# michalfratczak/habdec

Measured on AMD Instinct MI355X. Metric: IQ Msamples/s (batched 2.048 MS/s streams), higher is better.
Workload: dtype f32

## Files before the change

habdec_amd/capi.py:

```python
from __future__ import annotations

import ctypes as C
from pathlib import Path

import numpy as np

LIB_PATH = Path(__file__).resolve().parent / "libhabdec_amd.so"
_lib = None


class HabdecError(RuntimeError):
    pass


class hd_engine_config(C.Structure):
    _fields_ = [("device", C.c_int32), ("n_streams", C.c_uint32), ("max_chunk", C.c_uint32), ("sampling_rate", C.c_double),
                ("decimation", C.c_uint32), ("baud", C.c_double), ("rtty_bits", C.c_uint32), ("rtty_stops", C.c_float),
                ("lowpass_bw_hz", C.c_float), ("lowpass_trans", C.c_float), ("dc_remove", C.c_int32), ("lookup_mode", C.c_int32),
                ("enable_spectrum", C.c_int32), ("ungated", C.c_int32), ("keep_filtered", C.c_int32), ("pipeline", C.c_int32), ("arith", C.c_int32)]


class hd_afc_info(C.Structure):
    _fields_ = [("frequency_correction", C.c_double), ("shift_hz", C.c_double), ("noise_floor", C.c_double),
                ("noise_variance", C.c_double), ("peak_left", C.c_int32), ("peak_right", C.c_int32), ("spectra", C.c_uint64)]
# ... 40 lines not shown
    "hd_stream_set_dc_remove": (_int, [_vp, _u32, _int]),
    "hd_stream_reset_frequency_correction": (_int, [_vp, _u32, _dbl]),
    "hd_stream_set_tune": (_int, [_vp, _u32, _dbl]),
    "hd_stream_set_front_tune": (_int, [_vp, _u32, _dbl]),
    "hd_stream_front_tune": (_int, [_vp, _u32, C.POINTER(hd_front_tune_info)]),
    "hd_stream_set_auto_afc": (_int, [_vp, _u32, _int, _dbl, _dbl]),
    "hd_stream_tune": (_int, [_vp, _u32, C.POINTER(hd_tune_info)]),
    "hd_set_sentence_callback": (None, [_vp, SENTENCE_CB, _vp]),
    "hd_set_match_callback": (None, [_vp, MATCH_CB, _vp]),
    "hd_set_chars_callback": (None, [_vp, CHARS_CB, _vp]),
    "hd_process_host": (_int, [_vp, _vp, _sz, _vp, _u32]),
    "hd_process_device": (_int, [_vp, _vp, _sz, _vp, _u32]),
    "hd_flush": (_int, [_vp]),
    "hd_ingest_run": (_int, [_vp, _vp, C.c_uint64, C.POINTER(C.c_uint64)]),
    "hd_stream_rtty": (_sz, [_vp, _u32, C.c_char_p, _sz]),
    "hd_stream_last_sentence": (_sz, [_vp, _u32, C.c_char_p, _sz]),
    "hd_stream_take_sentences": (_sz, [_vp, _u32, C.c_char_p, _sz]),
    "hd_stream_take_matches": (_sz, [_vp, _u32, C.c_char_p, _sz]),
    "hd_stream_take_chars": (_sz, [_vp, _u32, C.c_char_p, _sz]),
    "hd_engine_sentences_ok": (C.c_uint64, [_vp]),
    "hd_stream_afc": (_int, [_vp, _u32, C.POINTER(hd_afc_info)]),
    "hd_stream_spectrum": (_sz, [_vp, _u32, _f32p, _sz]),
    "hd_stream_power": (_sz, [_vp, _u32, _f32p, _sz]),
    "hd_stream_demodulated": (_sz, [_vp, _u32, _f32p, _sz]),
    "hd_stream_decimated": (_sz, [_vp, _u32, _f32p, _sz]),
    "hd_stream_filtered": (_sz, [_vp, _u32, _f32p, _sz]),
    "hd_stream_bits": (_sz, [_vp, _u32, _u8p, _sz]),
    "hd_stream_flips": (_sz, [_vp, _u32, _u32p, _sz]),
    "hd_stream_fir_taps": (_sz, [_vp, _u32, _f32p, _sz]),
    "hd_stream_symbol_backlog": (_u32, [_vp, _u32]),
    "hd_stream_bits_total": (C.c_uint64, [_vp, _u32]),
    "hd_stream_flip_list_full": (C.c_uint64, [_vp, _u32]),
    "hd_stream_demod_checksum": (C.c_int, [_vp, _u32, C.POINTER(C.c_uint64), C.POINTER(C.c_uint32), C.POINTER(C.c_uint32)]),
    "hd_stream_demod_checksum_total": (C.c_int, [_vp, _u32, C.POINTER(C.c_uint64), C.POINTER(C.c_uint64), C.POINTER(C.c_uint64)]),
    "hd_min_chunk": (_u32, [_u32]),
    "hd_engine_timing": (_int, [_vp, C.POINTER(hd_timing)]),
    "hd_engine_set_timing": (None, [_vp, _int]),
}
HOST_API = {
    "hd_host_decim_plan": (_int, [C.c_uint, C.POINTER(_int), C.POINTER(C.c_uint)]),
    "hd_host_decim_taps": (_sz, [C.c_uint, _int, _f32p, _sz]),
    "hd_host_lowpass_design": (_sz, [_f, _f, _sz, _sz, _int, _f32p, _sz]),
    "hd_host_rtty_new": (_vp, [_sz, _f]),
    "hd_host_rtty_free": (None, [_vp]),
    "hd_host_rtty_pending": (_sz, [_vp]),
    "hd_host_rtty_push_run": (_sz, [_vp, _u8p, _sz, C.c_char_p, _sz]),
    "hd_host_crc16": (None, [C.c_char_p, _sz, C.c_char_p]),
    "hd_host_extract_sentence": (_int, [C.c_char_p, _sz, C.c_char_p, C.c_char_p, C.c_char_p, C.c_char_p, _sz]),
    "hd_host_text_new": (_vp, [_sz, _f]),
    "hd_host_text_free": (None, [_vp]),
    "hd_host_text_push_bits": (None, [_vp, _u8p, _sz]),
    "hd_host_text_get": (_sz, [_vp, _int, C.c_char_p, _sz]),
    "hd_host_afc_new": (_vp, []),
    "hd_host_afc_free": (None, [_vp]),
    "hd_host_afc_step": (None, [_vp, _int, _int, _int, _int, _f, _f, _dbl, _dbl, _sz, _dbl]),
    "hd_host_afc_reset": (None, [_vp, _dbl, _sz, _dbl]),
    "hd_host_afc_get": (None, [_vp] + [C.POINTER(_dbl)] * 4 + [C.POINTER(_int)] * 2),
    "hd_host_atan2f": (None, [_f32p, _f32p, _f32p, _sz]),
    "hd_host_discriminate": (None, [_f32p, _sz, _f, _f, _f32p]),
    "hd_host_spectrum_payload": (_sz, [_f32p, _sz, _dbl, _dbl, _dbl, _dbl, _int, _int, _f, _int, _int, _u8p, _sz, C.POINTER(_sz)]),
    "hd_host_demod_payload": (_sz, [_f32p, _sz, _int, _int, _u8p, _sz, C.POINTER(_sz)]),
    "hd_host_parse_time": (_int, [C.c_char_p, C.POINTER(_int), C.POINTER(_int), C.POINTER(_f)]),
    "hd_host_parse_gps_pos": (_int, [C.c_char_p, C.POINTER(_f)]),
    "hd_host_parse_sentence": (_int, [C.c_char_p, _vp]),
    "hd_host_timestamp_from_hms": (_sz, [C.c_int64, _int, _int, _f, C.c_char_p, _sz]),
    "hd_host_gps_distance": (None, [_dbl] * 6 + [C.POINTER(_dbl)]),
    "hd_host_sondehub_new": (_vp, [C.c_char_p, C.c_char_p]),
    "hd_host_sondehub_free": (None, [_vp]),
    "hd_host_sondehub_push_sentence": (_int, [_vp, _u32, C.c_char_p, C.c_char_p, C.c_int64]),
    "hd_host_sondehub_push": (_int, [_vp, C.c_char_p, C.c_char_p, C.c_char_p, _int, _f, _f, _f]),
    "hd_host_sondehub_size": (_sz, [_vp]),
    "hd_host_sondehub_take": (_sz, [_vp, C.c_int64, C.c_char_p, _sz, C.POINTER(_sz)]),
    "hd_host_utc_iso": (_sz, [C.c_int64, C.c_char_p, _sz]),
    "hd_host_json_number": (_sz, [_dbl, C.c_char_p, _sz]),
    "hd_host_iqfiles_open": (_vp, [C.POINTER(C.c_char_p), C.c_uint32, _int, C.c_uint32, C.c_uint32, _dbl]),
    "hd_host_iqfiles_close": (None, [_vp]),
    "hd_host_iqfiles_streams": (C.c_uint32, [_vp]),
    "hd_host_iqfiles_count": (C.c_uint64, [_vp, C.c_uint32]),
    "hd_host_iqfiles_rewinds": (C.c_uint64, [_vp, C.c_uint32]),
    "hd_host_iqfiles_next": (C.c_uint32, [_vp, _f32p, _sz, C.POINTER(C.c_uint32)]),
    "hd_host_tune_step": (_int, [_dbl, _dbl, C.POINTER(C.c_uint32)]),
    "hd_host_tune_tables": (None, [_f32p, _f32p]),
    "hd_host_tune_rotate": (None, [_f32p, _sz, C.c_uint32, C.c_uint32, _f32p]),
}


def lib() -> C.CDLL:
    global _lib
    if _lib is None:
        if not LIB_PATH.exists():
            raise HabdecError(f"{LIB_PATH} is missing: build it with `python -m habdec_amd.build` (hipcc, gfx950). "
                              "habdec_amd has no CPU or PyTorch fallback for the data path.")
        L = C.CDLL(str(LIB_PATH))
        for table in (ENGINE_API, HOST_API):
            for name, (res, args) in table.items():
                f = getattr(L, name)
                f.restype, f.argtypes = res, args
        _lib = L
    return _lib


def check(rc: int) -> None:
    if rc != 0:
        raise HabdecError(f"habdec_amd error {rc}: {lib().hd_last_error().decode()}")
```

habdec_amd/csrc/dev_types.h:

```cpp
#pragma once
#include <stdint.h>
#ifndef __HIPCC__
#ifndef __host__
#define __host__
#define __device__
#endif
#endif

namespace hd {

constexpr int kFftBins = 4096;
constexpr uint32_t kVentLimit = 30000;
constexpr uint32_t kFirBatch = 256;

struct StreamCall {
    uint32_t n_in;
    uint32_t n1;
    uint32_t n2;
    uint32_t zero_hist1;
    uint32_t zero_hist2;
    uint32_t pend_before;
    uint32_t fft_fill;
    uint32_t fft_take;
    uint32_t fft_run;
    uint32_t fir_m;
    uint32_t fir_taps;
    uint32_t fir_zero_hist;
    uint32_t pend_after;
    uint32_t dc_remove;
    uint32_t clear_pending;
    uint32_t fir_taps_prev;
};
__host__ __device__ inline uint32_t sc_taps_prev(const StreamCall& c) { return c.fir_taps_prev & 0xFFFFu; }
__host__ __device__ inline uint32_t sc_head_n(const StreamCall& c) { return (c.fir_taps_prev >> 16) & 0x3FFFu; }
__host__ __device__ inline bool sc_head_prev(const StreamCall& c) { return (c.fir_taps_prev >> 30) & 1u; }
__host__ __device__ inline bool sc_head_save(const StreamCall& c) { return (c.fir_taps_prev >> 31) & 1u; }
__host__ __device__ inline uint32_t sc_pack_taps_prev(uint32_t taps_prev, uint32_t head_n, bool head_prev, bool head_save)
{ return (taps_prev & 0xFFFFu) | ((head_n & 0x3FFFu) << 16) | ((head_prev ? 1u : 0u) << 30) | ((head_save ? 1u : 0u) << 31); }


struct SymbolParams {
    uint32_t spb;
    uint32_t R;
    uint32_t min_held;
    uint32_t float_abs;
    uint32_t reset;
};

struct SymState {
    uint32_t base;
    uint32_t held;
    uint32_t cached;
    uint32_t run_pos;
    float    run_sum;
    uint32_t _pad[3];
};

struct BitsHeader {
    uint32_t nbits;
    uint32_t held_after;
    uint32_t nflips;
    uint32_t overflow;
    uint32_t uncached;
    uint32_t demod_ck[2];
    uint32_t demod_n;
    uint32_t seq;
    uint32_t _pad[3];
};
static_assert(sizeof(BitsHeader) == 48, "result slot header");

struct SpectrumStatsDev {
    int32_t valid;
    int32_t peak1, peak2;
    float power1, power2;
    uint32_t seq;
    double mean, sigma;
};

}
```

habdec_amd/csrc/engine.cpp:

```cpp
#include <hip/hip_runtime.h>
#include <rocfft/rocfft.h>

#include <algorithm>
#include <atomic>
#include <chrono>
#include <cmath>
#include <cstdio>
#include <cstdlib>
#include <cstring>
#include <memory>
#include <condition_variable>
#include <mutex>
#include <thread>
#include <string>
#include <vector>

#include "../../include/habdec_amd.h"
#include "dev_types.h"
#include "host/afc_tracker.hpp"
#include "host/decim_plan.hpp"
#include "host/fir_design.hpp"
#include "host/iq_file_batch.hpp"
#include "host/text_stage.hpp"
#include "host/tune_host.hpp"
// ... 44 lines not shown
struct SizeState {
    size_t stage_buf[2] = {0, 0};
    size_t pending = 0;
    size_t fft_fill = 0;
    size_t fir_buf = 0;
    uint32_t fir_T_run = 0;
    uint32_t head_n = 0;
    uint64_t head_call = ~0ull;
    bool head_aside = false;
    uint32_t tune_phase = 0;
    uint32_t front_phase = 0;
    uint32_t win_ub = 0, inflight_m = 0;
    uint32_t last_n2 = 0, last_pend_before = 0, last_m = 0;
    int last_buf = 0;
};

struct StreamHost {
    double baud = 300;
    float lp_bw = 1500, lp_trans = 0.025f;
    bool dc = false;
    hd::LowpassDesigner lp;
    bool taps_dirty = false;
    uint32_t tune_step = 0;
    uint32_t held = 0;
    bool sym_reset = true;
    hd::TextStage text;
    hd::AfcTracker afc;
    hd::SpectrumStats stats{};
    bool have_spectrum = false;
    uint64_t spectra = 0;
    uint32_t last_nbits = 0, last_nflips = 0;
    uint64_t flip_list_full = 0;
    uint64_t bits_total = 0;
    std::vector<uint32_t> last_words;
    uint32_t demod_ck[2] = {0, 0}, demod_ck_n = 0xFFFFFFFFu;
    uint64_t demod_ck_call = 0;
    uint64_t demod_ck_hash = 0xCBF29CE484222325ull;
    uint64_t demod_ck_calls = 0, demod_ck_unknown = 0;
    double tune_hz = 0;
    uint64_t tune_from = 0, retunes = 0;
    bool auto_afc = false;
    double afc_hold_s = 6.0, afc_min_hz = 100.0;
    uint64_t afc_elapsed = 0;
    double front_hz = 0;
    uint32_t front_step = 0;
    uint64_t front_from = 0;
};

}

struct hd_engine {
    hd_engine_config cfg{};
    double fs = 0, fsd = 0;
    std::vector<hd::DecimStage> stages;
    uint32_t S = 0, D = 1;
    uint32_t n1_cap = 0, n2_cap = 0;
    uint32_t taps_cap = 0, fir_hist_cap = 0;
    size_t fbuf_stride = 0;
    uint32_t tail_cap = 0, backlog_cap = 0, slot_words = 0, flips_cap = 0, max_R = 0, min_R = 4;
    int bins_sep = 8;
    bool decode_enabled = true;
    bool fast = false;
    bool one_stream = false;
    bool no_tail = false;
    uint32_t tail_max_n2 = 2048;
    int last_route = -1;
    struct PendingTail { bool valid = false; hd::TailArgs ta{}; int slot = 0; int r2 = 0, t2 = 0; } pend;
    DevBuf<float2> fft_tw;
    bool no_claim = false;
    uint32_t step_run = 0;
    bool no_cu_step = false;
    uint32_t ring_run = 0;
    uint32_t ring_short_pct = 25;
    static constexpr uint32_t kS1Loaders = 2;
#ifndef HD_S1_SLOTS_BATCH
#define HD_S1_SLOTS_BATCH 4
#endif
    static constexpr uint32_t kS1Slots = HD_S1_SLOTS_BATCH;
    PinBuf<unsigned int> ring_gave_up;
    std::string fail_cause;
    bool device_failed = false;
    uint64_t step_launches = 0;
    DevBuf<unsigned int> step_ctr;
    uint32_t pend_max_taps = 0;
    bool dec_wgs_forced = false;
#ifdef HD_TIMING_EXPERIMENT
    int cu_exp = 0;
#else
    static constexpr int cu_exp = 0;
#endif
    uint32_t n_cus = 0, dec_wgs_per_cu = 0;
    hipStream_t qa = nullptr, qb = nullptr, qc = nullptr;
    hipStream_t qh = nullptr;
    DevBuf<float2> staging2;
    hipEvent_t ev_copy[2] = {nullptr, nullptr}, ev_staging_free[2] = {nullptr, nullptr};
    bool staging_used[2] = {false, false};
    uint64_t host_calls = 0, host_calls_in_place = 0;
    uint32_t timing_every = 8;
    hd_timing last_timing{};
    static constexpr uint32_t kLpFftMinTaps = 1024;
    uint32_t lpf_N[2] = {0, 0};
    rocfft_plan lpf_fwd[2] = {nullptr, nullptr}, lpf_inv[2] = {nullptr, nullptr};
    rocfft_execution_info lpf_info = nullptr;
    DevBuf<char> lpf_workbuf;
    DevBuf<float2> lpf_x, lpf_k;
    PinBuf<uint32_t> lpf_ntaps;
    uint32_t lpf_k_N = 0;
    bool lpf_k_stale = true;
    uint64_t lpf_calls = 0;

    DevBuf<float2> staging, dec1, dec1b, dec1c, hist1[2], hist2[2], fbuf[3], fft_in, spec, filtered;
    DevBuf<float> stage_taps[2], lp_taps, power, demod, tail, weight;
    DevBuf<unsigned long long> flipmask;
    DevBuf<uint32_t> flips_dbg;
    DevBuf<hd::SymState> d_symstate;
    DevBuf<hd::DemodCarry> carry[2];
    DevBuf<float2> fir_head;
    DevBuf<float> tune_tab;
    DevBuf<uint32_t> demod_ck_acc;
    uint32_t head_cap = 0;
    DevBuf<hd::SymbolParams> d_sym;
    PinBuf<hd::SymbolParams> h_sym;
    static constexpr int kSlots = 4;
    struct CallSlot {
        DevBuf<hd::StreamCall> d_call;
        PinBuf<hd::StreamCall> h_call;
        PinBuf<uint32_t> h_slots;
        PinBuf<hd::SpectrumStatsDev> h_stats;
        PinBuf<uint2> h_tune;
        PinBuf<uint2> h_front;
        bool timed = false, timed_step = false;
        hipEvent_t ev_front = nullptr, ev_done = nullptr, ev_params = nullptr, ev_spec = nullptr, t0 = nullptr, t1 = nullptr, t2 = nullptr, t3 = nullptr;
        bool busy = false;
        uint32_t seq = 0;
        uint64_t total_in = 0;
        uint32_t r1 = 1;
        ~CallSlot() { for (hipEvent_t ev : {ev_front, ev_done, ev_params, ev_spec, t0, t1, t2, t3}) if (ev) (void)hipEventDestroy(ev); }
    } slot[kSlots];
    uint64_t calls = 0;
    uint64_t delivered = 0;
    int cur = 0;
    int hist_cur = 0;
    int carry_cur = 0;
    bool sym_dirty = true;

    std::vector<StreamHost> st;
    std::vector<SizeState> mirror, mirror_next;
    std::recursive_mutex mtx;
    bool in_callback = false;
    hd_sentence_cb sentence_cb = nullptr; void* sentence_user = nullptr;
    hd_match_cb match_cb = nullptr; void* match_user = nullptr;
    hd_chars_cb chars_cb = nullptr; void* chars_user = nullptr;
    uint64_t sentences_ok = 0;

    ~hd_engine()
    {
        for (rocfft_plan pl : {lpf_fwd[0], lpf_fwd[1], lpf_inv[0], lpf_inv[1]}) if (pl) rocfft_plan_destroy(pl);
        if (lpf_info) rocfft_execution_info_destroy(lpf_info);
        if (qa) (void)hipStreamDestroy(qa);
        if (qb && qb != qa) (void)hipStreamDestroy(qb);
        if (qc && qc != qa) (void)hipStreamDestroy(qc);
        if (qh) (void)hipStreamDestroy(qh);
        for (hipEvent_t ev : {ev_copy[0], ev_copy[1], ev_staging_free[0], ev_staging_free[1]}) if (ev) (void)hipEventDestroy(ev);
    }
};

namespace {

std::once_flag g_rocfft_once;

hd::SymbolParams symbol_params(const hd_engine* e, const StreamHost& s)
{
    hd::SymbolParams p{};
    p.float_abs = e->cfg.lookup_mode ? 1u : 0u;
    p.min_held = 0xFFFFFFFFu;
    p.spb = 0; p.R = 4;
    if (e->fsd > 0 && s.baud > 0) {
        const double spb = std::round(e->fsd / s.baud);
        if (spb >= 1 && spb < 1e9) {
            p.spb = (uint32_t)spb;
            p.R = (uint32_t)std::max(4, int(p.spb / 4));
            p.min_held = (uint32_t)std::ceil(e->fsd / s.baud * 3);
        }
    }
    return p;
}

float cutoff_rel(const hd_engine* e, const StreamHost& s) { return (float)(s.lp_bw / e->fsd); }

int check_stream(const hd_engine* e, uint32_t s)
{
    if (!e) return fail(HD_ERR_INVALID, "null engine");
    if (s >= e->S) return fail(HD_ERR_INVALID, "stream index out of range");
    return HD_OK;
}

}

extern "C" {

const char* hd_last_error(void) { return g_err.c_str(); }

uint32_t hd_min_chunk(uint32_t decimation)
{
    std::vector<hd::DecimStage> st;
    if (!hd::decim_plan(decimation, st)) return 0;
    uint64_t need = decimation ? decimation : 1;
    uint64_t r = 1;
    for (const auto& g : st) { need = std::max<uint64_t>(need, (uint64_t)(g.taps.size() - 1) * r); r *= (uint64_t)g.ratio; }
    const uint64_t d = decimation ? decimation : 1;
    return (uint32_t)((need + d - 1) / d * d);
}

void hd_engine_config_default(hd_engine_config* c)
// ... 24 lines not shown
    e->fsd = e->fs / (double)e->D;
    e->decode_enabled = cfg->ungated || !(e->fsd > 4 * 40e3);
    if (cfg->baud > 0 && e->fsd / cfg->baud < 3.5)
        return fail(HD_ERR_UNSUPPORTED, "symbol rate above a third of the decimated rate (fewer than 4 samples per bit): the symbol extractor's windows would overlap");
    {
        const float rel = (float)(500.0f / e->fsd);
        e->bins_sep = std::max(8, (int)std::round((double)rel * (double)hd::kFftBins));
    }

    int ndev = 0;
    if (hipGetDeviceCount(&ndev) != hipSuccess || ndev <= cfg->device || cfg->device < 0)
        return fail(HD_ERR_DEVICE, "no HIP device " + std::to_string(cfg->device) + " (this library has no CPU path)");
    HD_HIP(hipSetDevice(cfg->device));
    HD_HIP(hipStreamCreateWithFlags(&e->qa, hipStreamNonBlocking));
    e->one_stream = cfg->pipeline == 0;
    e->no_tail = getenv("HD_NO_TAIL") != nullptr;
    e->no_claim = getenv("HD_NO_CLAIM") != nullptr;
    if (const char* v = getenv("HD_STEP_RUN")) e->step_run = (uint32_t)atoi(v);
    e->no_cu_step = getenv("HD_NO_CU_STEP") != nullptr;
    if (const char* v = getenv("HD_RING_RUN")) e->ring_run = (uint32_t)atoi(v);
    if (const char* v = getenv("HD_RING_SHORT_PCT")) e->ring_short_pct = std::min<uint32_t>((uint32_t)atoi(v), 100u);
    if (const char* v = getenv("HD_TAIL_MAX_N2")) e->tail_max_n2 = (uint32_t)strtoul(v, nullptr, 0);
    {
        hipDeviceProp_t prop;
        HD_HIP(hipGetDeviceProperties(&prop, cfg->device));
        e->n_cus = (uint32_t)prop.multiProcessorCount;
        e->dec_wgs_per_cu = cfg->pipeline ? 6u : 8u;
        if (const char* v = getenv("HD_DEC_WGS_PER_CU")) { e->dec_wgs_per_cu = (uint32_t)atoi(v); e->dec_wgs_forced = true; }
#ifdef HD_TIMING_EXPERIMENT
        if (const char* v = getenv("HD_CU_EXP")) e->cu_exp = atoi(v);
#endif
    }
    for (hipEvent_t* ev : {&e->ev_copy[0], &e->ev_copy[1], &e->ev_staging_free[0], &e->ev_staging_free[1]}) HD_HIP(hipEventCreateWithFlags(ev, hipEventDisableTiming));
    if (e->one_stream) e->qb = e->qc = e->qa;
    else {
        if (!e->qb) HD_HIP(hipStreamCreateWithFlags(&e->qb, hipStreamNonBlocking));
        HD_HIP(hipStreamCreateWithFlags(&e->qc, hipStreamNonBlocking));
    }
    for (auto& sl : e->slot) {
        static const unsigned ev_flags = (unsigned)hipEventDisableSystemFence;
        HD_HIP(hipEventCreateWithFlags(&sl.ev_front, hipEventDisableTiming | ev_flags));
        HD_HIP(hipEventCreateWithFlags(&sl.ev_done, hipEventDisableTiming | ev_flags));
        HD_HIP(hipEventCreateWithFlags(&sl.ev_params, hipEventDisableTiming | ev_flags));
        HD_HIP(hipEventCreateWithFlags(&sl.ev_spec, hipEventDisableTiming | ev_flags));
        for (hipEvent_t* ev : {&sl.t0, &sl.t1, &sl.t2, &sl.t3}) HD_HIP(hipEventCreateWithFlags(ev, ev_flags));
    }

    const uint32_t S = e->S;
    const uint32_t r0 = e->stages.size() > 0 ? e->stages[0].ratio : 1;
    e->n1_cap = cfg->max_chunk / r0;
    e->n2_cap = cfg->max_chunk / e->D;
    const uint32_t m_cap = ((e->n2_cap + hd::kFirBatch - 1) / hd::kFirBatch) * hd::kFirBatch + hd::kFirBatch;
    e->taps_cap = (m_cap | 1u) + 1u;
    e->fir_hist_cap = (e->taps_cap + 1u) & ~1u;
    e->fbuf_stride = (size_t)e->fir_hist_cap + hd::kFirBatch + e->n2_cap + 2;
    e->fbuf_stride = (e->fbuf_stride + 1) & ~(size_t)1;
    e->backlog_cap = hd::kVentLimit + 1 + m_cap;
    e->tail_cap = 1u;
    while (e->tail_cap < hd::kVentLimit + 1 + m_cap + 1024) e->tail_cap <<= 1;

    e->st.resize(S);
    e->mirror.resize(S);
    e->mirror_next.resize(S);
    for (auto& s : e->st) {
        s.baud = cfg->baud; s.lp_bw = cfg->lowpass_bw_hz; s.lp_trans = cfg->lowpass_trans; s.dc = cfg->dc_remove != 0;
        s.text.framer.nbits = cfg->rtty_bits; s.text.framer.nstops = cfg->rtty_stops;
        s.lp.float_trig = cfg->lookup_mode != 0;
    }
    {
        const hd::SymbolParams p = symbol_params(e.get(), e->st[0]);
        const uint32_t spb = std::max<uint32_t>(p.spb, 1);
        uint32_t bits = 3u * e->backlog_cap / spb + 64u;
        bits = std::max<uint32_t>(256u, (bits + 31u) & ~31u);
        e->slot_words = (uint32_t)(sizeof(hd::BitsHeader) / 4) + bits / 32;
        e->max_R = std::max<uint32_t>(p.R, 4);
        e->min_R = e->max_R;
    }
    e->flips_cap = cfg->keep_filtered ? 256 : 0;

    HD_HIP(e->staging.alloc((size_t)S * cfg->max_chunk));
    if (e->stages.size() == 2) for (auto* b : {&e->dec1, &e->dec1b, &e->dec1c}) HD_HIP(b->alloc((size_t)S * e->n1_cap));
    HD_HIP(e->step_ctr.alloc(2 * 16 * 32 + 32));
    HD_HIP(e->ring_gave_up.alloc(4));
    e->ring_gave_up.p[0] = 0;
    if (!e->no_claim && e->n_cus % 32u == 0) {
        const uint32_t n_xcd = e->n_cus / 32u;
        HD_HIP(hipDeviceSynchronize());
        const uint32_t seen = HDK(probe_xcc_mask, e->qa, e->n_cus, e->step_ctr.p + 2 * 16 * 32);
        if (n_xcd > 16 || seen != (n_xcd >= 32 ? 0xFFFFFFFFu : (1u << n_xcd) - 1u)) e->no_claim = true;
    } else
        e->no_claim = true;
    if (e->stages.size() >= 1) {
        for (auto& h : e->hist1) HD_HIP(h.alloc((size_t)S * (e->stages[0].taps.size() - 1)));
        HD_HIP(e->stage_taps[0].alloc(e->stages[0].taps.size() + 1));
        HD_HIP(hipMemcpy(e->stage_taps[0].p, e->stages[0].taps.data(), e->stages[0].taps.size() * 4, hipMemcpyHostToDevice));
    }
    if (e->stages.size() == 2) {
        for (auto& h : e->hist2) HD_HIP(h.alloc((size_t)S * (e->stages[1].taps.size() - 1)));
        HD_HIP(e->stage_taps[1].alloc(e->stages[1].taps.size() + 1));
        HD_HIP(hipMemcpy(e->stage_taps[1].p, e->stages[1].taps.data(), e->stages[1].taps.size() * 4, hipMemcpyHostToDevice));
    }
    for (auto& b : e->fbuf) HD_HIP(b.alloc((size_t)S * e->fbuf_stride));
    HD_HIP(e->lp_taps.alloc((size_t)S * e->taps_cap));
    HD_HIP(e->demod.alloc((size_t)S * m_cap));
    if (cfg->keep_filtered) HD_HIP(e->filtered.alloc((size_t)S * m_cap));
    HD_HIP(e->tail.alloc((size_t)S * e->tail_cap));
    HD_HIP(e->weight.alloc((size_t)S * e->tail_cap));
    HD_HIP(e->flipmask.alloc((size_t)S * (e->tail_cap / 64)));
    HD_HIP(e->d_symstate.alloc(S));
    if (e->flips_cap) HD_HIP(e->flips_dbg.alloc((size_t)S * e->flips_cap));
    for (auto& c : e->carry) HD_HIP(c.alloc(S));
    e->head_cap = std::min<uint32_t>(e->taps_cap, 8192u);
    HD_HIP(e->fir_head.alloc((size_t)S * e->head_cap));
    HD_HIP(e->demod_ck_acc.alloc((size_t)2 * S));
    HD_HIP(e->d_sym.alloc(S));
    HD_HIP(e->h_sym.alloc(S));
    for (auto& sl : e->slot) {
        HD_HIP(sl.d_call.alloc(S));
        HD_HIP(sl.h_call.alloc(S));
        HD_HIP(sl.h_slots.alloc((size_t)S * e->slot_words));
        HD_HIP(sl.h_tune.alloc(S));
        HD_HIP(sl.h_front.alloc(S));
    }
    {
        std::vector<float> tab(4 * hd::kTuneTable);
        hd::tune_tables(tab.data(), tab.data() + 2 * hd::kTuneTable);
        HD_HIP(e->tune_tab.alloc(tab.size()));
        HD_HIP(hipMemcpy(e->tune_tab.p, tab.data(), tab.size() * sizeof(float), hipMemcpyHostToDevice));
    }
    if (cfg->enable_spectrum) {
        HD_HIP(e->fft_in.alloc((size_t)S * hd::kFftBins));
        HD_HIP(e->spec.alloc((size_t)S * hd::kFftBins));
        HD_HIP(e->power.alloc((size_t)S * hd::kFftBins));
        for (auto& sl : e->slot) HD_HIP(sl.h_stats.alloc(S));
        {
            std::vector<float2> tw(hd::kFftBins);
            for (size_t m = 0; m < hd::kFftBins; ++m) {
                const double a = 2.0 * 3.14159265358979323846264338327950288 * (double)m / (double)hd::kFftBins;
                tw[m] = make_float2((float)std::cos(a), (float)-std::sin(a));
            }
            HD_HIP(e->fft_tw.alloc(hd::kFftBins));
            HD_HIP(hipMemcpy(e->fft_tw.p, tw.data(), tw.size() * sizeof(float2), hipMemcpyHostToDevice));
        }
    }
    if (e->fast && e->taps_cap >= hd_engine::kLpFftMinTaps && getenv("HD_NO_LP_FFT") == nullptr) {
        std::call_once(g_rocfft_once, [] { rocfft_setup(); });
        uint32_t N = 1;
        while (N < m_cap + e->taps_cap) N <<= 1;
        e->lpf_N[1] = N; e->lpf_N[0] = N / 2;
        size_t wmax = 0;
        for (int w = 0; w < 2; ++w) {
            const size_t len = e->lpf_N[w];
            if (rocfft_plan_create(&e->lpf_fwd[w], rocfft_placement_inplace, rocfft_transform_type_complex_forward, rocfft_precision_single, 1, &len, S, nullptr) != rocfft_status_success ||
                rocfft_plan_create(&e->lpf_inv[w], rocfft_placement_inplace, rocfft_transform_type_complex_inverse, rocfft_precision_single, 1, &len, S, nullptr) != rocfft_status_success)
                return fail(HD_ERR_DEVICE, "rocfft_plan_create (low-pass transforms) failed");
            for (rocfft_plan pl : {e->lpf_fwd[w], e->lpf_inv[w]}) { size_t wsz = 0; rocfft_plan_get_work_buffer_size(pl, &wsz); wmax = std::max(wmax, wsz); }
        }
        if (rocfft_execution_info_create(&e->lpf_info) != rocfft_status_success) return fail(HD_ERR_DEVICE, "rocfft_execution_info_create failed");
        if (wmax) { HD_HIP(e->lpf_workbuf.alloc(wmax)); rocfft_execution_info_set_work_buffer(e->lpf_info, e->lpf_workbuf.p, wmax); }
        HD_HIP(e->lpf_x.alloc((size_t)S * N));
        HD_HIP(e->lpf_k.alloc((size_t)S * N));
        HD_HIP(e->lpf_ntaps.alloc(S));
    }
    {
        hd_engine::CallSlot& sl = e->slot[0];
        hipStream_t q = e->qa;
// ... 138 lines not shown
int hd_stream_set_tune(hd_engine* e, uint32_t s, double offset_hz)
{
    if (int r = check_stream(e, s)) return r;
    std::lock_guard<std::recursive_mutex> l(e->mtx);
    uint32_t d = 0;
    if (!hd::tune_step(offset_hz, e->fsd, &d)) return fail(HD_ERR_INVALID, "tuning offset outside (-fs_dec/2, fs_dec/2)");
    StreamHost& st = e->st[s];
    st.tune_hz = offset_hz; st.tune_step = d; st.tune_from = e->calls;
    if (offset_hz == 0) e->mirror[s].tune_phase = 0;
    return HD_OK;
}
int hd_stream_set_front_tune(hd_engine* e, uint32_t s, double offset_hz)
{
    if (int r = check_stream(e, s)) return r;
    std::lock_guard<std::recursive_mutex> l(e->mtx);
    if (e->stages.empty()) return fail(HD_ERR_UNSUPPORTED, "an engine without a decimation stage has no input-rate tuning: hd_stream_set_tune is the same thing there");
    uint32_t d = 0;
    if (!hd::tune_step(offset_hz, e->fs, &d)) return fail(HD_ERR_INVALID, "tuning offset outside (-fs/2, fs/2)");
    StreamHost& st = e->st[s];
    st.front_hz = offset_hz; st.front_step = d; st.front_from = e->calls;
    if (offset_hz == 0) e->mirror[s].front_phase = 0;
    return HD_OK;
}
int hd_stream_front_tune(hd_engine* e, uint32_t s, hd_front_tune_info* out)
{
    if (int r = check_stream(e, s)) return r;
    if (!out) return fail(HD_ERR_INVALID, "null argument");
    std::lock_guard<std::recursive_mutex> l(e->mtx);
    const StreamHost& st = e->st[s];
    out->offset_hz = st.front_hz; out->step = st.front_step; out->phase = e->mirror[s].front_phase; out->from_call = st.front_from;
    return HD_OK;
}
int hd_stream_set_auto_afc(hd_engine* e, uint32_t s, int on, double hold_s, double min_hz)
{
    if (int r = check_stream(e, s)) return r;
    if (!(hold_s >= 0) || !(min_hz >= 0)) return fail(HD_ERR_INVALID, "hold_s and min_hz must be >= 0");
    std::lock_guard<std::recursive_mutex> l(e->mtx);
    StreamHost& st = e->st[s];
    st.auto_afc = on != 0; st.afc_hold_s = hold_s; st.afc_min_hz = min_hz; st.afc_elapsed = 0;
    return HD_OK;
}
int hd_stream_tune(hd_engine* e, uint32_t s, hd_tune_info* out)
{
    if (int r = check_stream(e, s)) return r;
    if (!out) return fail(HD_ERR_INVALID, "null argument");
    std::lock_guard<std::recursive_mutex> l(e->mtx);
    const StreamHost& st = e->st[s];
    out->offset_hz = st.tune_hz; out->step = st.tune_step; out->phase = e->mirror[s].tune_phase;
    out->retunes = st.retunes; out->from_call = st.tune_from; out->auto_afc = st.auto_afc ? 1 : 0;
    return HD_OK;
}

}


namespace {

int run_pending_tail(hd_engine* e)
{
    if (!e->pend.valid) return HD_OK;
    hd_engine::CallSlot& ps = e->slot[e->pend.slot];
    e->pend.valid = false;
    hd::TailArgs ta = e->pend.ta;
    const int lanes = (e->S >= 2 * e->n_cus ? 64 : 256);
    hd::TailArgs lay = ta;
    if (lanes != 64) {
        if (!HDK(tail_layout, lay, lanes, e->pend.r2, e->pend.t2, e->pend_max_taps, e->max_R, e->min_R, e->tail_cap, e->pend.ta.pend_max, 64 * 1024)) return fail(HD_ERR_INVALID, "stream tail layout");
    }
    if (!HDK(launch_tail, e->qa, lanes, e->pend.r2, e->pend.t2, e->S, lay, ps.ev_done)) return fail(HD_ERR_INVALID, "stream tail refused a shape it was selected for");
    HD_HIP(hipGetLastError());
    return HD_OK;
}

int collect(hd_engine* e, hd_engine::CallSlot& sl)
{
    if (!sl.busy) return HD_OK;
    if (e->pend.valid && &e->slot[e->pend.slot] == &sl) { if (const int r = run_pending_tail(e)) return r; }
    const auto w0 = std::chrono::steady_clock::now();
    HD_HIP(hipEventSynchronize(sl.ev_done));
    const auto w1 = std::chrono::steady_clock::now();
    sl.busy = false;
    if (sl.timed) {
        float a = 0, b = 0;
        HD_HIP(hipEventElapsedTime(&b, sl.t1, sl.t2));
        if (sl.timed_step) a = b; else HD_HIP(hipEventElapsedTime(&a, sl.t0, sl.t3));
        e->last_timing.ms_total = a;
        e->last_timing.ms_front = b;
        e->last_timing.samples = sl.total_in;
        e->last_timing.front_bytes = sl.total_in * 8 + (sl.total_in / sl.r1) * 8;
        ++e->last_timing.timed_calls;
    }
    int rc = HD_OK;
    {
        const auto t_lim = std::chrono::steady_clock::now() + std::chrono::milliseconds(200);
        const bool timing_experiment = e->cu_exp != 0;
        auto await = [&](const volatile uint32_t* tag, const char* what, uint32_t s) {
            for (uint32_t spins = 0; *tag != sl.seq; ++spins) {
                if (std::chrono::steady_clock::now() > t_lim) {
                    e->device_failed = true;
                    e->fail_cause = std::string(what) + " of stream " + std::to_string(s) + " does not carry its call's tag 200 ms after the completion event";
                    rc = fail(HD_ERR_DEVICE, e->fail_cause + ": the results of this engine are unreliable -- destroy the engine");
                    return;
                }
                if (spins > 64u) std::this_thread::yield();
            }
        };
        for (uint32_t s = 0; s < e->S && !e->device_failed && !timing_experiment; ++s) {
            await(&reinterpret_cast<const volatile hd::BitsHeader*>(sl.h_slots.p + (size_t)s * e->slot_words)->seq, "result slot", s);
            if (!e->device_failed && e->cfg.enable_spectrum && sl.h_stats.p && sl.h_call.p[s].fft_run)
                await(reinterpret_cast<const volatile uint32_t*>(&sl.h_stats.p[s].seq), "spectrum statistics", s);
        }
        std::atomic_thread_fence(std::memory_order_acquire);
    }
    if (e->ring_gave_up.p && e->ring_gave_up.p[0] && !e->device_failed) {
        e->device_failed = true;
        e->fail_cause = "k_stage1_cu (loader / consumer waves): a bounded wait ran out inside a launch (word " + std::to_string(e->ring_gave_up.p[0]) + ")";
    }
    if (e->device_failed && rc == HD_OK)
        rc = fail(HD_ERR_DEVICE, e->fail_cause + ": the results of this and of every later call of this engine are unreliable -- destroy the engine");
    if (e->device_failed) {
        e->last_timing.host_wait_us = std::chrono::duration<double, std::micro>(w1 - w0).count();
        e->last_timing.host_text_us = 0;
        return rc;
    }
    for (uint32_t s = 0; s < e->S; ++s) {
        StreamHost& st = e->st[s];
        const hd::StreamCall& c = sl.h_call.p[s];
        if (c.fft_run) {
            std::memcpy(&st.stats, &sl.h_stats.p[s], sizeof(st.stats));
            st.have_spectrum = true;
            ++st.spectra;
        }
        const bool past_batch_gate = c.fir_m || c.clear_pending;
        if (past_batch_gate && e->cfg.enable_spectrum) st.afc.step(st.have_spectrum, st.stats, hd::kFftBins, e->fsd);
        st.afc_elapsed += c.n_in;
        if (st.auto_afc && (double)st.afc_elapsed >= st.afc_hold_s * e->fs && std::abs(st.afc.correction) > st.afc_min_hz) {
            const double corr = st.afc.correction;
            uint32_t d = 0;
            if (hd::tune_step(st.tune_hz + corr, e->fsd, &d)) {
                st.tune_hz += corr; st.tune_step = d; st.tune_from = e->calls;
                if (!d) e->mirror[s].tune_phase = 0;
                st.afc.reset(corr, hd::kFftBins, e->fsd);
                st.afc_elapsed = 0;
                ++st.retunes;
            }
        }
        const uint32_t* slot = sl.h_slots.p + (size_t)s * e->slot_words;
        const hd::BitsHeader* hdr = reinterpret_cast<const hd::BitsHeader*>(slot);
        SizeState& sz = e->mirror[s];
        st.held = hdr->held_after;
        sz.inflight_m -= c.fir_m;
        sz.win_ub = hdr->uncached + sz.inflight_m;
        st.last_nbits = hdr->nbits; st.last_nflips = hdr->nflips;
        st.bits_total += hdr->nbits;
        st.demod_ck[0] = hdr->demod_ck[0]; st.demod_ck[1] = hdr->demod_ck[1]; st.demod_ck_n = hdr->demod_n; st.demod_ck_call = e->delivered;
        if (hdr->demod_n != 0xFFFFFFFFu) {
            for (const uint32_t x : {hdr->demod_n, hdr->demod_ck[0], hdr->demod_ck[1]}) st.demod_ck_hash = (st.demod_ck_hash ^ x) * 0x100000001B3ull;
            ++st.demod_ck_calls;
        } else ++st.demod_ck_unknown;
        if (hdr->overflow & 1u) rc = fail(HD_ERR_CAPACITY, "symbol result slot overflow on stream " + std::to_string(s));
        if (hdr->overflow & 2u) ++st.flip_list_full;
        const uint32_t* words = slot + sizeof(hd::BitsHeader) / 4;
        st.last_words.assign(words, words + (hdr->nbits + 31) / 32);
        if (!c.fir_m) continue;
        if (hdr->nbits) st.text.framer.push_packed(words, hdr->nbits);
        const std::string chars = st.text.run(hdr->nbits != 0, [&](const hd::SentenceMatch& m) {
            ++e->sentences_ok;
// ... 158 lines not shown
    const uint32_t step_lds = (p.R1 == 32 || p.R1 == 64) ? HDK(step_lds_bytes, (int)p.R1, (int)p.T1) : 0u;
    const bool step = tail && !p.any_front && e->cfg.pipeline && !e->one_stream && p.min_in == p.max_in && p.max_in && step_lds &&
                      HDK(tail_layout, r.ta_step, 64, R2, T2, p.max_taps, e->max_R, e->min_R, e->tail_cap, p.max_pend, step_lds);
    r.route = step ? Route::step : tail ? Route::tail : Route::separate;
    r.any_post = p.any_dc || (p.any_tune && !tail);
    r.lean = tail && !e->one_stream;
    r.free_front = !tail && p.nst == 2 && !e->one_stream;
    r.host_params = tail && !step && e->one_stream;
    r.dcall = r.host_params ? sl.h_call.dev : sl.d_call.p;
    r.feed = (e->cfg.enable_spectrum && !r.any_post) ? e->fft_in.p : nullptr;
    if (r.route != Route::separate || !e->cfg.enable_spectrum || r.any_post || !p.any_fft) return;
    for (uint32_t s = 0; s < S; ++s) {
        hd::StreamCall& c = sl.h_call.p[s];
        if (c.fft_run == 1 && c.fft_fill == 0 && c.fft_take == (uint32_t)hd::kFftBins) { c.fft_take = 0; c.fft_run = 2; }
    }
    r.spectrum_on_qc = !e->one_stream && p.nst != 0;
    for (uint32_t s = 0; s < S && r.spectrum_on_qc; ++s) r.spectrum_on_qc = sl.h_call.p[s].fft_run != 1u;
}

void fill_tail(const hd_engine* e, const hd_engine::CallSlot& sl, const CallPlan& p, const CallRoute& r, const CallBufs& b, hd::TailArgs& t)
{
    t.dec1 = b.d1; t.dec1_stride = e->n1_cap; t.hist2_in = e->hist2[b.hin].p; t.hist2_out = e->hist2[b.hout].p; t.taps2 = e->stage_taps[1].p;
    t.fbuf = b.fcur; t.fbuf_next = b.fnext; t.fbuf_stride = e->fbuf_stride; t.fir_hist_cap = e->fir_hist_cap;
    t.lp_taps = e->lp_taps.p; t.taps_stride = e->taps_cap; t.demod = e->demod.p; t.demod_stride = e->demod.n / e->S;
    t.filtered = e->cfg.keep_filtered ? e->filtered.p : nullptr; t.carry_in = e->carry[b.cin].p; t.carry_out = e->carry[b.cout].p;
    t.tune = p.any_tune ? sl.h_tune.dev : nullptr; t.tune_tab = e->tune_tab.p;
    t.call = r.dcall; t.fft_in = r.feed; t.head_buf = e->fir_head.p; t.fbuf_prev = b.fprev; t.head_cap = e->head_cap;
    t.n_streams = e->S;
    t.ring = e->tail.p; t.ring_cap = e->tail_cap; t.sym = e->d_symstate.p; t.flipmask = e->flipmask.p; t.wsum = e->weight.p;
    t.sp = e->d_sym.p; t.slots = sl.h_slots.dev; t.slot_words = e->slot_words; t.seq = sl.seq;
    t.flips_dbg = e->flips_cap ? e->flips_dbg.p : nullptr; t.flips_cap = e->flips_cap;
    t.fft_tw = r.feed ? e->fft_tw.p : nullptr;
    t.spec = e->spec.p; t.power = e->power.p; t.stats = sl.h_stats.dev; t.rate = e->fsd; t.bins_sep = e->bins_sep;
}

hd::StepClaim make_claim(const hd_engine* e, const CallPlan& p, uint32_t lin_wgs ,
                         uint32_t run_len_cu )
{
    hd::StepClaim claim{};
    const int R1 = (int)p.R1, T1 = (int)p.T1;
    const uint64_t S = e->S;
    const uint32_t ntiles = run_len_cu ? HDK(ring_tiles, R1, T1, p.max_in) : (p.max_n1 + 63) / 64, n_xcd = e->n_cus / 32u, run_len = run_len_cu ? run_len_cu : e->step_run >= 2 ? e->step_run : 4u;
    const uint64_t runs = S * ntiles / run_len;
    const bool shape_ok = run_len_cu ? (HDK(stage1_cu_supported, R1, T1) && p.max_in % 2048u == 0) : ((R1 == 32 || R1 == 64) && p.max_n1 % 64 == 0);
    if (!e->no_claim && (p.nst == 2 || (run_len_cu && p.nst == 1)) && shape_ok && p.min_in == p.max_in && p.max_in && !p.any_zero1 && n_xcd && e->n_cus % 32u == 0 && n_xcd <= 16 &&
        ntiles && (ntiles % run_len == 0 || (run_len_cu && R1 >= 32 && (S * ntiles) % run_len == 0)) && runs % n_xcd == 0 && S * ntiles < (1ull << 32) && (uint64_t)ntiles * S >= 4ull * lin_wgs) {
        claim.ctr = e->step_ctr.p + (size_t)(e->step_launches & 1u) * 16 * 32;
        claim.ctr_next = e->step_ctr.p + (size_t)((e->step_launches & 1u) ^ 1u) * 16 * 32;
        claim.n_xcd = n_xcd; claim.runs_per_xcd = (uint32_t)(runs / n_xcd); claim.run_len = run_len;
        if (run_len_cu && R1 >= 32 && e->ring_short_pct) {
            const uint32_t tpx = claim.runs_per_xcd * run_len, whole = (uint32_t)((uint64_t)tpx * (100u - e->ring_short_pct) / 100u) / run_len;
            claim.tiles_per_xcd = tpx; claim.short_from = whole; claim.runs_per_xcd = whole + (tpx - whole * run_len);
        }
    }
    return claim;
}

uint32_t pick_ring_run(const hd_engine* e, uint32_t R1, uint32_t ntiles)
{
    const uint64_t S = e->S;
    const uint32_t n_xcd = e->n_cus / 32u ? e->n_cus / 32u : 1u, want = R1 >= 32 ? 4u : 8u;
    auto ok = [&](uint32_t r) { return r >= 2u && r <= ntiles && (R1 >= 32 ? (S * ntiles) % r == 0 : ntiles % r == 0) && (S * ntiles / r) % n_xcd == 0; };
    if (e->ring_run >= 2 && ok(e->ring_run)) return e->ring_run;
    for (uint32_t d = 0; d <= 8u; ++d) {
        if (ok(want + d)) return want + d;
        if (d && d < want && ok(want - d)) return want - d;
    }
    return 2u;
}

int enqueue_uploads(hd_engine* e, hd_engine::CallSlot& sl, const CallRoute& r)
{
    const uint32_t S = e->S;
    hipStream_t qa = e->qa;
    if (e->last_route >= 0 && e->last_route != (int)r.route) {
        if (const int rc = run_pending_tail(e)) return rc;
        HD_HIP(hipStreamSynchronize(qa)); HD_HIP(hipStreamSynchronize(e->qb));
    }
    e->last_route = (int)r.route;
    e->last_timing.path = (uint32_t)r.route;
    if (!r.lean && !r.free_front && e->calls >= 2 && !e->one_stream) HD_HIP(hipStreamWaitEvent(qa, e->slot[(e->calls - 2) % hd_engine::kSlots].ev_done, 0));
    const bool step = r.route == Route::step;
    sl.timed = e->timing_every && (e->calls % e->timing_every) == 0;
    sl.timed_step = sl.timed && step;
    if (sl.timed && !step) HD_HIP(hipEventRecord(sl.t0, qa));
    if (!r.lean && !r.free_front && !r.host_params) {
        HDK(launch_fetch_params, e->qc, sl.h_call.dev, sl.d_call.p, S * sizeof(hd::StreamCall));
        if (!e->one_stream) { HD_HIP(hipEventRecord(sl.ev_params, e->qc)); HD_HIP(hipStreamWaitEvent(qa, sl.ev_params, 0)); }
    }
    for (uint32_t s = 0; s < S; ++s) {
        StreamHost& st = e->st[s];
        if (!st.taps_dirty) continue;
        HD_HIP(hipMemcpyAsync(e->lp_taps.p + (size_t)s * e->taps_cap, st.lp.taps.data(), st.lp.taps.size() * 4, hipMemcpyHostToDevice, qa));
        st.taps_dirty = false;
        e->lpf_k_stale = true;
    }
    if (e->sym_dirty) {
        uint32_t mr = 4;
        for (uint32_t s = 0; s < S; ++s) {
            e->h_sym.p[s] = symbol_params(e, e->st[s]);
            e->h_sym.p[s].reset = e->st[s].sym_reset ? 1u : 0u;
            mr = std::max(mr, e->h_sym.p[s].R);
        }
        e->max_R = mr;
        { uint32_t lo = mr; for (uint32_t s2 = 0; s2 < S; ++s2) lo = std::min(lo, std::max<uint32_t>(e->h_sym.p[s2].R, 4)); e->min_R = lo; }
        HD_HIP(hipMemcpyAsync(e->d_sym.p, e->h_sym.p, S * sizeof(hd::SymbolParams), hipMemcpyHostToDevice, qa));
        e->sym_dirty = false;
        for (uint32_t s = 0; s < S; ++s)
            if (e->st[s].sym_reset) { e->st[s].sym_reset = false; e->sym_dirty = true; }
    }
    return HD_OK;
}

int enqueue_step(hd_engine* e, hd_engine::CallSlot& sl, const CallPlan& p, CallRoute& r, const float2* iq, size_t stride)
{
    const uint32_t S = e->S;
    const int R1 = (int)p.R1, T1 = (int)p.T1, R2 = (int)p.R2, T2 = (int)p.T2;
    hipStream_t qa = e->qa;
    const CallBufs b = call_bufs(e);
    const uint32_t ring_nt = HDK(ring_tiles, R1, T1, p.max_in), ring_run = pick_ring_run(e, p.R1, ring_nt), n_xcd = e->n_cus / 32u;
    const bool runs_ok = ring_nt && n_xcd && ring_run >= 2u && ((uint64_t)S * ring_nt) % ring_run == 0 && ((uint64_t)S * ring_nt / ring_run) % n_xcd == 0;
    const bool cu_shape = !e->no_cu_step && !e->no_claim && !p.any_zero1 && p.max_in % 2048u == 0 && runs_ok && HDK(step_cu_supported, R1, T1, R2, T2);
    const uint32_t cu_tail = cu_shape ? HDK(step_cu_tail_lds, R1, T1) : 0u;
    if (cu_tail) {
        hd::TailArgs tacu{};
        if (HDK(tail_layout, tacu, 64, R2, T2, p.max_taps, e->max_R, e->min_R, e->tail_cap, p.max_pend, cu_tail)) r.ta_step = tacu;
    }
    fill_tail(e, sl, p, r, b, r.ta_step);
    hd_engine::PendingTail prev = e->pend;
    hd_engine::CallSlot* ps = prev.valid ? &e->slot[prev.slot] : nullptr;
    const int cu_exp = e->cu_exp;
    const bool want_cu = cu_tail && ((cu_exp & 1) || (r.ta_step.lds_bytes <= cu_tail && (!prev.valid || prev.ta.lds_bytes <= cu_tail)));
    const hd::StepClaim claim = make_claim(e, p, 0, want_cu ? ring_run : 0u);
    bool launched = false;
    if (want_cu && claim.ctr) {
        const uint32_t tb = std::max(r.ta_step.lds_bytes, prev.valid ? prev.ta.lds_bytes : 0u);
        hd::StepClaim cl = claim;
        if (cu_exp & 2) { cl.runs_per_xcd = 0; cl.tiles_per_xcd = 0; cl.short_from = 0xFFFFFFFFu; }
        launched = HDK(launch_step_cu, qa, R1, T1, prev.valid ? prev.r2 : R2, prev.valid ? prev.t2 : T2, S, e->n_cus, iq, stride,
                                      e->hist1[b.hin].p, e->hist1[b.hout].p, e->stage_taps[0].p, b.d1, e->n1_cap, sl.h_call.dev, sl.d_call.p, prev.ta,
                                      (prev.valid && !(cu_exp & 1)) ? S : 0u, p.max_in, cl, tb,
                                      sl.timed ? sl.t1 : nullptr, sl.timed ? sl.t2 : ps ? ps->ev_done : nullptr);
    }
    e->last_timing.step_variant = launched ? 1u : 0u;
    if (launched) ++e->step_launches;
    else {
        if (sl.timed) HD_HIP(hipEventRecord(sl.t1, qa));
        const hd::StepClaim fb = (want_cu && claim.ctr) ? hd::StepClaim{} : claim;
        const uint32_t wgs = (fb.ctr ? 8u : 32u) * e->n_cus;
        if (prev.valid && prev.ta.lds_bytes > HDK(step_lds_bytes, R1, T1)) {
            if (const int rc = run_pending_tail(e)) return rc;
            prev.valid = false; ps = nullptr;
        }
        if (!HDK(launch_step, qa, R1, T1, prev.valid ? prev.r2 : R2, prev.valid ? prev.t2 : T2, S, p.max_n1, iq, stride, e->hist1[b.hin].p,
                             e->hist1[b.hout].p, e->stage_taps[0].p, b.d1, e->n1_cap, sl.h_call.dev, sl.d_call.p, wgs, prev.ta, prev.valid ? S : 0u,
                             p.any_zero1 ? 0u : p.max_in, fb))
            return fail(HD_ERR_INVALID, "no step kernel for this decimation plan");
        if (fb.ctr) ++e->step_launches;
    }
    if (sl.timed && !launched) HD_HIP(hipEventRecord(sl.t2, qa));
    if (ps && (!launched || sl.timed)) HD_HIP(hipEventRecord(ps->ev_done, qa));
    HD_HIP(hipGetLastError());
    return HD_OK;
}

void call_spectrum(hd_engine* e, hipStream_t q, hd_engine::CallSlot& sl, const CallPlan& p, const CallRoute& r)
{
    if (!(e->cfg.enable_spectrum && p.max_n2)) return;
    const float2* fcur = e->fbuf[e->cur].p;
    if (r.any_post || p.nst == 0) HDK(launch_fft_feed, q, e->S, fcur, e->fbuf_stride, e->fft_in.p, r.dcall, e->fir_hist_cap);
    if (!p.any_fft) return;
    hd::launch_spectrum_wave(q, e->S, e->fft_in.p, e->fft_tw.p, e->spec.p, e->power.p, sl.h_stats.dev, r.dcall, e->fsd, e->bins_sep, sl.seq, fcur, e->fbuf_stride, e->fir_hist_cap);
}

int enqueue_front(hd_engine* e, hd_engine::CallSlot& sl, const CallPlan& p, const CallRoute& r, const float2* iq, size_t stride)
{
    const uint32_t S = e->S, R1 = p.R1, T1 = p.T1;
    const bool tail = r.route == Route::tail;
    hipStream_t qa = e->qa;
    const CallBufs b = call_bufs(e);
    if (p.nst == 0) {
        if (sl.timed) HD_HIP(hipEventRecord(sl.t1, qa));
        HDK(launch_passthrough, qa, S, p.max_in, iq, stride, b.fcur, e->fbuf_stride, r.dcall, e->fir_hist_cap);
        if (sl.timed) HD_HIP(hipEventRecord(sl.t2, qa));
    } else {
        const bool single = p.nst == 1;
        float2* out1 = single ? b.fcur : b.d1;
        const size_t out1_stride = single ? e->fbuf_stride : e->n1_cap;
        const uint32_t wgs_cu = (R1 == 64 && !e->dec_wgs_forced && e->dec_wgs_per_cu > 4u) ? 4u : e->dec_wgs_per_cu;
        const uint32_t lin1 = (p.min_in == p.max_in && p.max_in) ? wgs_cu * e->n_cus : 0u;
        bool s1_cu = false;
        if (!p.any_front && (single ? R1 == 4 : R1 != 4) && p.min_in == p.max_in && p.max_in && !e->no_cu_step && !p.any_zero1 && p.max_in % 2048u == 0 && HDK(stage1_cu_supported, (int)R1, (int)T1)) {
            const hd::StepClaim cl = make_claim(e, p, 0, pick_ring_run(e, R1, HDK(ring_tiles, (int)R1, (int)T1, p.max_in)));
            if (cl.ctr) {
                if (sl.timed) HD_HIP(hipEventRecord(sl.t1, qa));
                s1_cu = HDK(launch_stage1_cu, qa, (int)R1, (int)T1, e->n_cus, iq, stride, e->hist1[b.hin].p, e->hist1[b.hout].p, e->stage_taps[0].p, out1, out1_stride,
                                             p.max_in, cl, e->ring_gave_up.dev, hd_engine::kS1Loaders, 16u, (e->cfg.pipeline && !tail && !single) ? hd_engine::kS1Slots : 8u,
                                             single ? r.dcall : nullptr, e->fir_hist_cap, single ? r.feed : nullptr);
                if (s1_cu) ++e->step_launches;
            }
        }
        e->last_timing.step_variant = s1_cu ? 1u : 0u;
        if (!s1_cu) {
            if (sl.timed) HD_HIP(hipEventRecord(sl.t1, qa));
            const hd::StreamCall* call1 = (r.lean || r.free_front) ? sl.h_call.dev : r.dcall;
            if (!(p.any_front ? HDK(launch_decimate_tuned, qa, R1, T1, S, p.max_n1, iq, stride, e->hist1[b.hin].p, e->hist1[b.hout].p, e->stage_taps[0].p, out1, out1_stride,
                                                          call1, single ? 1 : 0, e->fir_hist_cap, single ? r.feed : nullptr, lin1, sl.h_front.dev, e->tune_tab.p)
                              : HDK(launch_decimate, qa, R1, T1, S, p.max_n1, iq, stride, e->hist1[b.hin].p, e->hist1[b.hout].p, e->stage_taps[0].p, out1, out1_stride,
                                                    call1, 0, single ? 1 : 0, e->fir_hist_cap, single ? r.feed : nullptr, lin1)))
                return fail(HD_ERR_INVALID, "no kernel for this decimation stage");
        }
        if (sl.timed) HD_HIP(hipEventRecord(sl.t2, qa));
        if (r.free_front) HDK(launch_fetch_params, qa, sl.h_call.dev, sl.d_call.p, S * sizeof(hd::StreamCall));
        if (!single && !tail) {
            if (!HDK(launch_decimate, qa, p.R2, p.T2, S, p.max_n2, b.d1, e->n1_cap, e->hist2[b.hin].p, e->hist2[b.hout].p, e->stage_taps[1].p, b.fcur,
                                     e->fbuf_stride, r.dcall, 1, 1, e->fir_hist_cap, r.feed))
                return fail(HD_ERR_INVALID, "no kernel for this decimation stage");
        }
    }
    if (!tail) {
        if (r.any_post) HDK(launch_chunk_post, qa, S, b.fcur, e->fbuf_stride, r.dcall, e->fir_hist_cap, p.any_tune ? sl.h_tune.dev : nullptr, e->tune_tab.p);
        if (!r.spectrum_on_qc) call_spectrum(e, qa, sl, p, r);
    }
    if (!e->one_stream) HD_HIP(hipEventRecord(sl.ev_front, qa));
    if (r.spectrum_on_qc) {
        HD_HIP(hipStreamWaitEvent(e->qc, sl.ev_front, 0));
        call_spectrum(e, e->qc, sl, p, r);
        HD_HIP(hipEventRecord(sl.ev_spec, e->qc));
    }
    return HD_OK;
}

int lowpass_transforms(hd_engine* e, const CallPlan& p, const CallRoute& r, const CallBufs& b, uint32_t* lpN)
{
    *lpN = 0;
    if (!e->fast || !e->lpf_N[1] || p.max_taps < hd_engine::kLpFftMinTaps || !p.max_m || p.any_lp_restart) return HD_OK;
    const uint32_t S = e->S, Lmax = p.max_m + p.max_taps - 1;
    const int w = Lmax <= e->lpf_N[0] ? 0 : Lmax <= e->lpf_N[1] ? 1 : -1;
    if (w < 0) return HD_OK;
    const uint32_t N = e->lpf_N[w];
    hipStream_t qb = e->qb;
    rocfft_execution_info_set_stream(e->lpf_info, qb);
    if (e->lpf_k_stale || e->lpf_k_N != N) {
        for (uint32_t s = 0; s < S; ++s) e->lpf_ntaps.p[s] = (uint32_t)e->st[s].lp.taps.size();
// ... 411 lines not shown
```

habdec_amd/csrc/host_api.cpp:

```cpp
#include <algorithm>
#include <cstring>
#include <string>

#include "../../include/habdec_amd_host.h"
#include "host/afc_tracker.hpp"
#include "host/decim_plan.hpp"
#include "host/fir_design.hpp"
#include "host/gui_payload.hpp"
#include "host/telemetry.hpp"
#include "host/sondehub.hpp"
#include "host/text_stage.hpp"
#include "host/iq_file_batch.hpp"
#include "host/tune_host.hpp"
#include "kernels/exact_math.h"

struct hd_host_rtty { hd::RttyFramer f; };
struct hd_host_text { hd::TextStage t; };
struct hd_host_afc { hd::AfcTracker a; };

static void put(char* dst, size_t cap, const std::string& s)
{
    if (!dst || !cap) return;
    const size_t n = std::min(cap - 1, s.size());
    std::memcpy(dst, s.data(), n);
    dst[n] = 0;
}

extern "C" {

int hd_host_decim_plan(unsigned total, int ratio[2], unsigned ntaps[2])
{
    std::vector<hd::DecimStage> st;
    if (!hd::decim_plan(total, st)) return -1;
    for (size_t i = 0; i < st.size(); ++i) { ratio[i] = st[i].ratio; ntaps[i] = (unsigned)st[i].taps.size(); }
    return (int)st.size();
}
size_t hd_host_decim_taps(unsigned total, int stage, float* taps, size_t cap)
{
    std::vector<hd::DecimStage> st;
    if (!hd::decim_plan(total, st) || stage < 0 || (size_t)stage >= st.size()) return 0;
    const auto& t = st[stage].taps;
    std::memcpy(taps, t.data(), std::min(cap, t.size()) * sizeof(float));
    return t.size();
}
size_t hd_host_lowpass_design(float cutoff_rel, float transition, size_t batch, size_t prev_ntaps, int float_trig, float* taps, size_t cap)
{
    hd::LowpassDesigner d;
    d.float_trig = float_trig != 0;
    d.batch = batch;
    d.taps.assign(prev_ntaps, 0.0f);
    if (!d.design(cutoff_rel, transition)) return 0;
    std::memcpy(taps, d.taps.data(), std::min(cap, d.taps.size()) * sizeof(float));
    return d.taps.size();
}

hd_host_rtty* hd_host_rtty_new(size_t nbits, float nstops) { auto* r = new hd_host_rtty; r->f.nbits = nbits; r->f.nstops = nstops; return r; }
void hd_host_rtty_free(hd_host_rtty* r) { delete r; }
size_t hd_host_rtty_pending(const hd_host_rtty* r) { return r ? r->f.pending() : 0; }
size_t hd_host_rtty_push_run(hd_host_rtty* r, const uint8_t* bits, size_t n, char* out, size_t cap)
{
    r->f.push_bits(bits, n);
    std::string s;
    r->f.frame(s);
    std::memcpy(out, s.data(), std::min(cap, s.size()));
    return s.size();
}

void hd_host_crc16(const char* s, size_t n, char out4[5])
{
    const std::string r = hd::crc16_ccitt_hex(std::string(s, n));
    std::memcpy(out4, r.c_str(), 5);
}
int hd_host_extract_sentence(const char* stream, size_t n, char* callsign, char* data, char* crc, char* rest, size_t cap)
{
    hd::SentenceMatch m;
    if (!hd::extract_sentence(std::string(stream, n), m)) return 0;
    put(callsign, cap, m.callsign); put(data, cap, m.data); put(crc, cap, m.crc); put(rest, cap, m.rest);
    return 1;
}

hd_host_text* hd_host_text_new(size_t nbits, float nstops) { auto* t = new hd_host_text; t->t.framer.nbits = nbits; t->t.framer.nstops = nstops; return t; }
void hd_host_text_free(hd_host_text* t) { delete t; }
void hd_host_text_push_bits(hd_host_text* t, const uint8_t* bits, size_t n)
{
    if (n) t->t.framer.push_bits(bits, n);
    t->t.run(n != 0, [](const hd::SentenceMatch&) {});
}
size_t hd_host_text_get(hd_host_text* t, int which, char* buf, size_t cap)
{
    const std::string* s = &t->t.stream;
    if (which == 1) s = &t->t.last_sentence; else if (which == 2) s = &t->t.ok_log; else if (which == 3) s = &t->t.match_log; else if (which == 4) s = &t->t.char_log;
    put(buf, cap, *s);
    return s->size();
}

hd_host_afc* hd_host_afc_new(void) { return new hd_host_afc; }
void hd_host_afc_free(hd_host_afc* a) { delete a; }
// ... 67 lines not shown
size_t hd_host_timestamp_from_hms(int64_t now_unix, int hour, int minute, float second, char* buf, size_t cap)
{
    const std::string s = hd::telemetry::timestamp_from_hms(now_unix, hour, minute, second);
    if (buf && cap) { const size_t n = std::min(cap - 1, s.size()); std::memcpy(buf, s.data(), n); buf[n] = 0; }
    return s.size();
}
void hd_host_gps_distance(double lat1, double lon1, double alt1, double lat2, double lon2, double alt2, double out[5])
{
    const auto d = hd::telemetry::gps_distance(lat1, lon1, alt1, lat2, lon2, alt2);
    out[0] = d.line; out[1] = d.circle; out[2] = d.radians; out[3] = d.elevation_deg; out[4] = d.bearing_deg;
}

struct hd_host_sondehub {
    hd::SondehubBatch b;
    std::string pending;
    size_t pending_n = 0;
    hd_host_sondehub(const char* u, const char* v) : b(u ? u : "", v ? v : "") {}
};
hd_host_sondehub* hd_host_sondehub_new(const char* uploader_callsign, const char* software_version) { return new hd_host_sondehub(uploader_callsign, software_version); }
void hd_host_sondehub_free(hd_host_sondehub* h) { delete h; }
int hd_host_sondehub_push_sentence(hd_host_sondehub* h, uint32_t stream, const char* callsign, const char* data, int64_t now_unix_ns)
{
    if (!h || !callsign || !data) return -1;
    return h->b.push_sentence(stream, callsign, data, now_unix_ns);
}
int hd_host_sondehub_push(hd_host_sondehub* h, const char* payload_callsign, const char* time_received, const char* datetime, int frame, float lat, float lon, float alt)
{
    if (!h || !payload_callsign || !time_received || !datetime) return -1;
    hd::SondeRecord r;
    r.payload_callsign = payload_callsign; r.time_received = time_received; r.datetime = datetime; r.frame = frame; r.lat = lat; r.lon = lon; r.alt = alt;
    h->b.push(r);
    return 1;
}
size_t hd_host_sondehub_size(const hd_host_sondehub* h) { return h ? h->b.size() : 0; }
size_t hd_host_sondehub_take(hd_host_sondehub* h, int64_t now_unix_ns, char* out, size_t cap, size_t* n_records)
{
    if (!h) return 0;
    if (h->pending.empty()) h->pending = h->b.take(now_unix_ns, &h->pending_n);
    const size_t n = h->pending.size();
    if (n_records) *n_records = h->pending_n;
    if (out && cap > n) { std::memcpy(out, h->pending.data(), n); out[n] = 0; h->pending.clear(); h->pending_n = 0; }
    return n;
}
size_t hd_host_utc_iso(int64_t unix_ns, char* buf, size_t cap)
{
    const std::string s = hd::utc_iso_ns(unix_ns);
    if (buf && cap) { const size_t n = std::min(cap - 1, s.size()); std::memcpy(buf, s.data(), n); buf[n] = 0; }
    return s.size();
}
size_t hd_host_json_number(double v, char* buf, size_t cap)
{
    const std::string s = hd::json_number(v);
    if (buf && cap) { const size_t n = std::min(cap - 1, s.size()); std::memcpy(buf, s.data(), n); buf[n] = 0; }
    return s.size();
}

hd_host_iqfiles* hd_host_iqfiles_open(const char* const* paths, uint32_t n_files, int loop, uint32_t chunk, uint32_t granule, double realtime_rate)
{
    if (!paths || !n_files) return nullptr;
    std::vector<std::string> v;
    for (uint32_t i = 0; i < n_files; ++i) { if (!paths[i]) return nullptr; v.emplace_back(paths[i]); }
    auto* h = new hd_host_iqfiles;
    if (!h->batch.open(v, loop != 0, chunk, granule, realtime_rate)) { delete h; return nullptr; }
    return h;
}
void hd_host_iqfiles_close(hd_host_iqfiles* h) { delete h; }
uint32_t hd_host_iqfiles_streams(const hd_host_iqfiles* h) { return h ? h->batch.streams() : 0; }
uint64_t hd_host_iqfiles_count(const hd_host_iqfiles* h, uint32_t stream) { return (h && stream < h->batch.streams()) ? h->batch.file(stream).count() : 0; }
uint64_t hd_host_iqfiles_rewinds(const hd_host_iqfiles* h, uint32_t stream) { return (h && stream < h->batch.streams()) ? h->batch.file(stream).rewinds() : 0; }
uint32_t hd_host_iqfiles_next(hd_host_iqfiles* h, float* slab, size_t stride, uint32_t* n_per_stream)
{
    if (!h || !slab || !n_per_stream || stride < h->batch.chunk()) return 0;
    return h->batch.next(slab, stride, n_per_stream);
}

int hd_host_tune_step(double offset_hz, double decimated_rate, uint32_t* step)
{
    uint32_t d = 0;
    if (!hd::tune_step(offset_hz, decimated_rate, &d)) return -1;
    if (step) *step = d;
    return 0;
}
void hd_host_tune_tables(float coarse[512], float fine[512]) { hd::tune_tables(coarse, fine); }
void hd_host_tune_rotate(const float* iq, size_t n, uint32_t phase, uint32_t step, float* out)
{
    float tab[4 * hd::kTuneTable];
    hd::tune_tables(tab, tab + 2 * hd::kTuneTable);
    hd::tune_rotate(tab, iq, n, phase, step, out);
}

}
```

habdec_amd/csrc/kernels/decimate.hip:

```cpp
#include <hip/hip_runtime.h>
#include <hip/hip_ext.h>
#include <type_traits>
#include <cstdlib>

#include "launch.h"
#include "tune.h"
#include "tail_body.h"
#include "stage1_ring.h"

#ifndef HD_FRONT_SWEEPS
#define HD_FRONT_SWEEPS 2
#endif
#define HD_DEC_MAXW 4

namespace hd {
namespace HD_ARITH_NS {

#ifdef HD_STAMP_DEC
#ifndef HD_STAMP_DEC_D
#define HD_STAMP_DEC_D 32
#endif
__device__ unsigned long long g_dec_stamps[4096 * 8];
extern "C" void HD_DBG_NAME(hd_debug_dec_stamps)(unsigned long long* host, size_t n) { (void)hipMemcpyFromSymbol(host, HIP_SYMBOL(g_dec_stamps), n * 8); }
#define DSTAMP_DECL unsigned long long ds_t = __builtin_amdgcn_s_memtime(), ds_acc[4] = {0, 0, 0, 0}; const unsigned long long ds_r0 = __builtin_amdgcn_s_memrealtime(); unsigned long long ds_r1 = 0
// ... 436 lines not shown
                leave_copy(s);
            }
        }
        if (jump) {
            __syncthreads();
            s = jump_s; tile_i = jump_first; jump = false;
            if constexpr (TUNED) ft.tn = ftune[s];
            if (!tile_i) leave_copy(s);
        }
    }
    store_prev();
    flush_copy();
    DSTAMP_WRITE();
}

template <int D, int T, int TO>
__global__ __launch_bounds__(TO) __attribute__((amdgpu_waves_per_eu(D == 64 ? 1 : 2, TO == 64 ? 2 : HD_DEC_MAXW))) void k_decimate(const float2* __restrict__ in, size_t in_stride,
                                                   const float2* __restrict__ hist_in, float2* __restrict__ hist_out,
                                                   const float* __restrict__ taps,
                                                   float2* __restrict__ out, size_t out_stride,
                                                   const StreamCall* __restrict__ call, int stage, int final_stage,
                                                   uint32_t fir_hist_cap, uint32_t tiles_per_wg, float2* __restrict__ fft_in,
                                                   uint32_t n_streams, uint32_t lin_ntiles, StreamCall* __restrict__ call_copy,
                                                   const uint32_t uniform_n, const StepClaim claim)
{
    __shared__ float4 tile4[dec_tile_f4<D, T, TO>()];
    decimate_body<D, T, TO>(in, in_stride, hist_in, hist_out, taps, out, out_stride, call, stage, final_stage, fir_hist_cap, tiles_per_wg, fft_in,
                            n_streams, lin_ntiles, call_copy, blockIdx.x, blockIdx.y, gridDim.x, tile4, TO == 64 ? uniform_n : 0u,
                            TO == 64 ? claim : StepClaim{});
}

template <int TO> constexpr bool front_tab_in_lds()
{
#ifdef HD_FRONT_TAB_GLOBAL
    return false;
#else
    return TO > 64;
#endif
}

template <int D, int T, int TO>
__global__ __launch_bounds__(TO) __attribute__((amdgpu_waves_per_eu(D == 64 ? 1 : 2, TO == 64 ? 2 : HD_DEC_MAXW))) void k_decimate_tuned(const float2* __restrict__ in, size_t in_stride,
                                                   const float2* __restrict__ hist_in, float2* __restrict__ hist_out,
                                                   const float* __restrict__ taps,
                                                   float2* __restrict__ out, size_t out_stride,
                                                   const StreamCall* __restrict__ call, int final_stage,
                                                   uint32_t fir_hist_cap, uint32_t tiles_per_wg, float2* __restrict__ fft_in,
                                                   uint32_t n_streams, uint32_t lin_ntiles,
                                                   const uint2* __restrict__ ftune, const float* __restrict__ ftab)
{
    constexpr bool kLds = front_tab_in_lds<TO>();
    __shared__ float4 tile4[dec_tile_f4<D, T, TO>()];
    __shared__ float4 tab4[kLds ? kTuneTable : 1];
    if constexpr (kLds) {
        for (uint32_t i = threadIdx.x; i < kTuneTable; i += TO) tab4[i] = reinterpret_cast<const float4*>(ftab)[i];
        __syncthreads();
    }
    decimate_body<D, T, TO, true>(in, in_stride, hist_in, hist_out, taps, out, out_stride, call, 0, final_stage, fir_hist_cap, tiles_per_wg, fft_in,
                                  n_streams, lin_ntiles, nullptr, blockIdx.x, blockIdx.y, gridDim.x, tile4, 0u, StepClaim{}, ftune,
                                  kLds ? reinterpret_cast<const float*>(tab4) : ftab);
}

template <int D, int T, int D2, int T2>
__global__ __launch_bounds__(64) __attribute__((amdgpu_waves_per_eu(D == 64 ? 1 : 2, 2))) void k_step(const float2* __restrict__ in, size_t in_stride,
                                                   const float2* __restrict__ hist_in, float2* __restrict__ hist_out,
                                                   const float* __restrict__ taps,
                                                   float2* __restrict__ out, size_t out_stride,
                                                   const StreamCall* __restrict__ call, uint32_t n_streams, uint32_t lin_ntiles,
                                                   StreamCall* __restrict__ call_copy, const TailArgs ta, const uint32_t n_tail,
                                                   const uint32_t uniform_n, const StepClaim claim)
{
    constexpr int kF4 = dec_tile_f4<D, T, 64>() > (int)(kStepLdsBytes / 16) ? dec_tile_f4<D, T, 64>() : (int)(kStepLdsBytes / 16);
    __shared__ float4 tile4[kF4];
    if (blockIdx.x < n_tail) {
#define HD_STEP_PRIO 3
        __builtin_amdgcn_s_setprio(HD_STEP_PRIO);
        tail_body<64, 4, D2, T2>(ta, blockIdx.x, reinterpret_cast<unsigned char*>(tile4));
        return;
    }
    decimate_body<D, T, 64>(in, in_stride, hist_in, hist_out, taps, out, out_stride, call, 0, 0, 0u, 0u, nullptr, n_streams, lin_ntiles, call_copy,
                            blockIdx.x - n_tail, 0u, gridDim.x - n_tail, tile4, uniform_n, claim);
}

template <int T, int D2, int T2>
__global__ __launch_bounds__(512) void k_step_cu(const RingArgs ra, const StreamCall* __restrict__ call, StreamCall* __restrict__ call_copy,
                                                 const TailArgs ta, const uint32_t n_tail, const uint32_t n_streams, const uint32_t tail_bytes )
{
    extern __shared__ __attribute__((aligned(16))) unsigned char cu_lds[];
    RingCtl* ctl = reinterpret_cast<RingCtl*>(cu_lds);
    unsigned char* slots = cu_lds + kRingCtlBytes;
    unsigned char* tails = slots + 4 * kWorkSlotBytes;
    ring_ctl_init(ctl, 0u);
    __syncthreads();
    const uint32_t simd = (__builtin_amdgcn_s_getreg((2 - 1) << 11 | 4 << 6 | 4)) & 3u;
    uint32_t rank = 0;
    if ((threadIdx.x & 63u) == 0) rank = __hip_atomic_fetch_add(&ctl->simd_rank[simd], 1u, __ATOMIC_RELAXED, __HIP_MEMORY_SCOPE_WORKGROUP);
    rank = (uint32_t)__builtin_amdgcn_readfirstlane((int)rank);
    uint32_t w = rank ? 4u + simd : simd;
    if (rank < 2u && (threadIdx.x & 63u) == 0) (void)__hip_atomic_fetch_or(&ctl->roles_taken, 1u << w, __ATOMIC_RELAXED, __HIP_MEMORY_SCOPE_WORKGROUP);
    __syncthreads();
    if (rank >= 2u) {
        uint32_t pick = 0;
        if ((threadIdx.x & 63u) == 0) {
            for (;;) {
                const uint32_t taken = __hip_atomic_load(&ctl->roles_taken, __ATOMIC_RELAXED, __HIP_MEMORY_SCOPE_WORKGROUP);
                pick = (uint32_t)__builtin_ctz(~taken);
                if (!(__hip_atomic_fetch_or(&ctl->roles_taken, 1u << pick, __ATOMIC_RELAXED, __HIP_MEMORY_SCOPE_WORKGROUP) & (1u << pick))) break;
            }
        }
        w = (uint32_t)__builtin_amdgcn_readfirstlane((int)pick);
    }
    if (w < 4u) {
        ring_worker<T>(ra, slots + w * (uint32_t)kWorkSlotBytes, w);
    } else {
        const uint32_t k = w - 4u, lane = threadIdx.x & 63u;
        const uint32_t s = blockIdx.x * 4u + k;
        if (s < n_streams) {
            if (s < n_tail) {
                __builtin_amdgcn_s_setprio(HD_STEP_PRIO);
                tail_body<64, 4, D2, T2>(ta, s, tails + k * tail_bytes);
                __builtin_amdgcn_s_setprio(0);
            }
            if (call_copy && lane < 4) reinterpret_cast<uint4*>(call_copy + s)[lane] = reinterpret_cast<const uint4*>(call + s)[lane];
        }
        ring_worker<T>(ra, n_tail ? tails + k * tail_bytes : slots + w * (uint32_t)kWorkSlotBytes, w);
    }
}

template <int T, int D>
__global__ __launch_bounds__(D == 4 ? 1024 : D == 64 ? 256 : 512) void k_stage1_cu(const RingArgs ra, const uint32_t n_loaders, const uint32_t n_slots )
{
    extern __shared__ __attribute__((aligned(16))) unsigned char cu_lds[];
    if constexpr (D == 32 || D == 64) {
        ring_worker<T, D>(ra, cu_lds + (threadIdx.x >> 6) * (uint32_t)work_slot_bytes<D>(), threadIdx.x >> 6);
    } else {
    unsigned char* ring = cu_lds;
    RingCtl* ctl = reinterpret_cast<RingCtl*>(cu_lds + n_slots * ring_slot_bytes<T>());
    ring_ctl_init(ctl, n_loaders);
    __syncthreads();
    const uint32_t simd = (__builtin_amdgcn_s_getreg((2 - 1) << 11 | 4 << 6 | 4)) & 3u;
    uint32_t rank = 0;
    if ((threadIdx.x & 63u) == 0) rank = __hip_atomic_fetch_add(&ctl->simd_rank[simd], 1u, __ATOMIC_RELAXED, __HIP_MEMORY_SCOPE_WORKGROUP);
    rank = (uint32_t)__builtin_amdgcn_readfirstlane((int)rank);
    uint32_t w = simd < 2u ? (rank ? 2u + simd : simd) : 4u + 2u * (simd - 2u) + rank;
    if (rank < 2u && (threadIdx.x & 63u) == 0) (void)__hip_atomic_fetch_or(&ctl->roles_taken, 1u << w, __ATOMIC_RELAXED, __HIP_MEMORY_SCOPE_WORKGROUP);
    __syncthreads();
    if (rank >= 2u) {
        uint32_t pick = 0;
        if ((threadIdx.x & 63u) == 0) {
            for (;;) {
                const uint32_t taken = __hip_atomic_load(&ctl->roles_taken, __ATOMIC_RELAXED, __HIP_MEMORY_SCOPE_WORKGROUP);
                pick = (uint32_t)__builtin_ctz(~taken);
                if (!(__hip_atomic_fetch_or(&ctl->roles_taken, 1u << pick, __ATOMIC_RELAXED, __HIP_MEMORY_SCOPE_WORKGROUP) & (1u << pick))) break;
            }
        }
        w = (uint32_t)__builtin_amdgcn_readfirstlane((int)pick);
    }
    const RingGeom geom{ring, n_slots};
    const uint32_t h0 = n_slots / 2u;
    if (w < n_loaders) ring_loader<T>(ra, geom, ctl, (n_loaders == 1u || w == 0u) ? 0u : h0, n_loaders == 1u ? n_slots : (w == 0u ? h0 : n_slots - h0), w);
    else ring_consumer<T, D>(ra, geom, ctl, w == 2, w);
    }
}

__global__ void k_xcc_probe(unsigned int* mask)
{
    if (threadIdx.x == 0) atomicOr(mask, 1u << (__builtin_amdgcn_s_getreg((3 << 11) | (0 << 6) | 20) & 15u));
}

__global__ void k_passthrough(const float2* __restrict__ in, size_t in_stride, float2* __restrict__ out, size_t out_stride,
                              const StreamCall* __restrict__ call, uint32_t fir_hist_cap)
{
    const uint32_t s = blockIdx.y;
    const StreamCall c = call[s];
    const uint32_t i = blockIdx.x * blockDim.x + threadIdx.x;
    if (i < c.n_in) out[(size_t)s * out_stride + fir_hist_cap + c.pend_before + i] = in[(size_t)s * in_stride + i];
}

__global__ __launch_bounds__(64) void k_dc_remove(float2* __restrict__ fbuf, size_t stride, const StreamCall* __restrict__ call,
                                                   uint32_t fir_hist_cap, const uint2* __restrict__ tune, const float* __restrict__ tab)
{
    const uint32_t s = blockIdx.x;
    const StreamCall c = call[s];
    const uint2 tn = tune ? tune[s] : make_uint2(0u, 0u);
    const bool dc = c.dc_remove != 0, rot = tn.x != 0u;
    if (!c.n2 || !(dc || rot)) return;
    float2* x = fbuf + (size_t)s * stride + fir_hist_cap + c.pend_before;
    const int lane = threadIdx.x;
    const float2 x0 = x[0];
    float wr = 0.97f * x0.x, wi = 0.97f * x0.y;
    for (uint32_t base = 0; base < c.n2; base += 64) {
        const uint32_t i = base + lane;
        float2 v = i < c.n2 ? x[i] : make_float2(0.f, 0.f);
        float yr = v.x, yi = v.y;
        if (dc) {
            yr = 0.f; yi = 0.f;
#pragma unroll 8
            for (int k = 0; k < 64; ++k) {
                const float xr = __builtin_bit_cast(float, __builtin_amdgcn_readlane(__builtin_bit_cast(int, v.x), k));
                const float xi = __builtin_bit_cast(float, __builtin_amdgcn_readlane(__builtin_bit_cast(int, v.y), k));
                const float sr = 0.97f * wr, si = 0.97f * wi;
                const float nr = xr + sr, ni = xi + si;
                if (lane == k) { yr = nr - wr; yi = ni - wi; }
                if (base + k < c.n2) { wr = nr; wi = ni; }
            }
        }
        if (rot) tune_rotate1(tab, tn.y + i * tn.x, yr, yi, yr, yi);
        if (i < c.n2) x[i] = make_float2(yr, yi);
    }
// ... 29 lines not shown
    while (per < 16 && (uint64_t)((ntiles + 2 * per - 1) / (2 * per)) * n_streams >= 2048) per *= 2;
    dim3 grid((ntiles + per - 1) / per, n_streams);
    hipLaunchKernelGGL((k_decimate<D, T, TO>), grid, dim3(TO), 0, st, in, in_stride, hist_in, hist_out, taps, out, out_stride, call,
                       stage, final_stage, fir_hist_cap, per, fft_in, n_streams, 0u, (StreamCall*)nullptr, 0u, StepClaim{});
}

bool launch_decimate(hipStream_t st, int ratio, int ntaps, uint32_t n_streams, uint32_t max_out, const float2* in, size_t in_stride,
                     const float2* hist_in, float2* hist_out, const float* taps, float2* out, size_t out_stride, const StreamCall* call,
                     int stage, int final_stage, uint32_t fir_hist_cap, float2* fft_in, uint32_t lin_wgs, StreamCall* call_copy,
                     uint32_t uniform_n, const StepClaim& claim)
{
    if (!max_out) return true;
#define HD_CASE(D, T, TO) \
    if (ratio == D && ntaps == T) { launch_one<D, T, TO>(st, n_streams, max_out, in, in_stride, hist_in, hist_out, taps, out, out_stride, call, stage, final_stage, fir_hist_cap, fft_in, lin_wgs, call_copy, uniform_n, claim); return true; }
    HD_CASE(2, 69, 256) HD_CASE(4, 139, 256) HD_CASE(8, 280, 256) HD_CASE(8, 54, 256)
    HD_CASE(16, 107, 128) HD_CASE(32, 212, 64) HD_CASE(32, 174, 64) HD_CASE(64, 348, 64)
#undef HD_CASE
    return false;
}

bool launch_decimate_tuned(hipStream_t st, int ratio, int ntaps, uint32_t n_streams, uint32_t max_out, const float2* in, size_t in_stride,
                           const float2* hist_in, float2* hist_out, const float* taps, float2* out, size_t out_stride, const StreamCall* call,
                           int final_stage, uint32_t fir_hist_cap, float2* fft_in, uint32_t lin_wgs, const uint2* ftune, const float* ftab)
{
    if (!max_out) return true;
#define HD_CASE(D, T, TO) \
    if (ratio == D && ntaps == T) { launch_one<D, T, TO, true>(st, n_streams, max_out, in, in_stride, hist_in, hist_out, taps, out, out_stride, call, 0, final_stage, fir_hist_cap, fft_in, lin_wgs, nullptr, 0u, StepClaim{}, ftune, ftab); return true; }
    HD_CASE(2, 69, 256) HD_CASE(4, 139, 256) HD_CASE(8, 280, 256) HD_CASE(8, 54, 256)
    HD_CASE(16, 107, 128) HD_CASE(32, 212, 64) HD_CASE(32, 174, 64) HD_CASE(64, 348, 64)
#undef HD_CASE
    return false;
}

uint32_t step_lds_bytes(int ratio, int ntaps)
{
    auto sz = [](int f4) { return (uint32_t)(f4 > (int)(kStepLdsBytes / 16) ? f4 : (int)(kStepLdsBytes / 16)) * 16u; };
    if (ratio == 32 && ntaps == 212) return sz(dec_tile_f4<32, 212, 64>());
    if (ratio == 32 && ntaps == 174) return sz(dec_tile_f4<32, 174, 64>());
    if (ratio == 64 && ntaps == 348) return sz(dec_tile_f4<64, 348, 64>());
    return 0;
}

bool launch_step(hipStream_t st, int ratio, int ntaps, int ratio2, int ntaps2, uint32_t n_streams, uint32_t n_out, const float2* in, size_t in_stride,
                 const float2* hist_in, float2* hist_out, const float* taps, float2* out, size_t out_stride, const StreamCall* call,
                 StreamCall* call_copy, uint32_t stage1_wgs, const TailArgs& ta, uint32_t n_tail, uint32_t uniform_n, const StepClaim& claim)
{
#define HD_STEP_CASE(D, T, D2, T2)                                                                                                    \
    if (ratio == D && ntaps == T && ratio2 == D2 && ntaps2 == T2) {                                                                   \
        const uint32_t ntiles = (n_out + 63) / 64;                                                                                    \
        hipLaunchKernelGGL((k_step<D, T, D2, T2>), dim3(n_tail + stage1_wgs), dim3(64), 0, st, in, in_stride, hist_in, hist_out, taps, out, \
                           out_stride, call, n_streams, ntiles, call_copy, ta, n_tail, uniform_n, claim);                             \
        return true;                                                                                                                  \
    }
    HD_STEP_CASE(32, 212, 2, 69) HD_STEP_CASE(32, 174, 4, 139) HD_STEP_CASE(64, 348, 4, 139)
#undef HD_STEP_CASE
    return false;
}

uint32_t ring_tiles(int ratio, int ntaps, uint32_t n)
{
    if (ratio != 32 && ratio != 64) return n / 2048u;
    const uint32_t adv = 64u - (uint32_t)((ntaps - 1 + ratio - 1) / ratio), rows = n / (uint32_t)ratio;
    return rows >= 64u ? (rows + adv - 1u) / adv : 0u;
}

static bool ring_limits_ok(uint32_t ntiles, const StepClaim& claim, bool workers = false )
{
    const uint64_t total = claim.tiles_per_xcd ? (uint64_t)claim.tiles_per_xcd * claim.n_xcd : (uint64_t)claim.runs_per_xcd * claim.n_xcd * claim.run_len;
    if (workers) return ntiles && claim.run_len >= 2u && total % ntiles == 0 && total < (1ull << 32) &&
                        (!claim.tiles_per_xcd || (uint64_t)claim.tiles_per_xcd == (uint64_t)(claim.short_from < claim.runs_per_xcd ? claim.short_from : claim.runs_per_xcd) * claim.run_len +
                                                                                    (claim.runs_per_xcd - (claim.short_from < claim.runs_per_xcd ? claim.short_from : claim.runs_per_xcd)));
    return ntiles && ntiles <= 4096u && claim.run_len && ntiles % claim.run_len == 0 && total < (1ull << 24) && total / ntiles <= (1ull << 20);
}

uint32_t step_cu_tail_lds(int ratio, int ntaps)
{
    if (ratio != 32 || (ntaps != 212 && ntaps != 174)) return 0;
    return ((163840u - (uint32_t)kRingCtlBytes - 4u * (uint32_t)kWorkSlotBytes) / 4u) & ~15u;
}

bool launch_step_cu(hipStream_t st, int ratio, int ntaps, int ratio2, int ntaps2, uint32_t n_streams, uint32_t n_cus, const float2* in, size_t in_stride,
                    const float2* hist_in, float2* hist_out, const float* taps, float2* out, size_t out_stride, const StreamCall* call,
                    StreamCall* call_copy, const TailArgs& ta, uint32_t n_tail, uint32_t uniform_n, const StepClaim& claim, uint32_t tail_bytes,
                    hipEvent_t ev_start, hipEvent_t ev_stop)
{
    if (ratio != 32 || !claim.ctr || !uniform_n || uniform_n % 2048u) return false;
    const uint32_t ntiles = ring_tiles(ratio, ntaps, uniform_n);
    if (!ring_limits_ok(ntiles, claim, true)) return false;
    if (tail_bytes < (uint32_t)kWorkSlotBytes) tail_bytes = (uint32_t)kWorkSlotBytes;
    tail_bytes = (tail_bytes + 15u) & ~15u;
    RingArgs ra{in, in_stride, hist_in, hist_out, taps, out, out_stride, uniform_n, ntiles, claim, nullptr, nullptr, 0u, nullptr};
#define HD_CU_CASE(T, D2, T2)                                                                                                         \
    if (ntaps == T && ratio2 == D2 && ntaps2 == T2) {                                                                                 \
        const uint32_t lds = (uint32_t)kRingCtlBytes + (n_tail ? 4u * (uint32_t)kWorkSlotBytes + 4u * tail_bytes : 8u * (uint32_t)kWorkSlotBytes); \
        if (lds > 163840u) return false;                                                                                              \
        static bool attr_set[64] = {};                              \
        int dev_ = 0;                                                                                                                 \
        if (hipGetDevice(&dev_) != hipSuccess || dev_ < 0 || dev_ >= 64) return false;                                                \
        if (!attr_set[dev_]) {                                                                                                        \
            if (hipFuncSetAttribute(reinterpret_cast<const void*>(k_step_cu<T, D2, T2>), hipFuncAttributeMaxDynamicSharedMemorySize, 163840) != hipSuccess) return false; \
            attr_set[dev_] = true;                                                                                                    \
        }                                                                                                                             \
        const dim3 grid_(n_cus > (n_streams + 3u) / 4u ? n_cus : (n_streams + 3u) / 4u);                                             \
             \
        if (ev_start || ev_stop) hipExtLaunchKernelGGL((k_step_cu<T, D2, T2>), grid_, dim3(512), lds, st, ev_start, ev_stop, 0u, ra, call, call_copy, ta, n_tail, n_streams, tail_bytes); \
        else hipLaunchKernelGGL((k_step_cu<T, D2, T2>), grid_, dim3(512), lds, st, ra, call, call_copy, ta, n_tail, n_streams, tail_bytes); \
        return true;                                                                                                                  \
    }
    HD_CU_CASE(212, 2, 69) HD_CU_CASE(174, 4, 139)
#undef HD_CU_CASE
    return false;
}

bool step_cu_supported(int ratio, int ntaps, int ratio2, int ntaps2)
{
    return ratio == 32 && ((ntaps == 212 && ratio2 == 2 && ntaps2 == 69) || (ntaps == 174 && ratio2 == 4 && ntaps2 == 139));
}

bool stage1_cu_supported(int ratio, int ntaps)
{
    return (ratio == 32 && (ntaps == 212 || ntaps == 174)) || (ratio == 64 && ntaps == 348) || (ratio == 8 && ntaps == 54) || (ratio == 4 && ntaps == 139);
}

bool launch_stage1_cu(hipStream_t st, int ratio, int ntaps, uint32_t n_cus, const float2* in, size_t in_stride, const float2* hist_in, float2* hist_out,
                      const float* taps, float2* out, size_t out_stride, uint32_t uniform_n, const StepClaim& claim, unsigned int* gave_up, uint32_t n_loaders, uint32_t n_waves,
                      uint32_t n_slots, const StreamCall* final_call, uint32_t fir_hist_cap, float2* fft_in)
{
    if (n_loaders != 1u) n_loaders = 2u;
    if (ratio <= 4) {
        n_loaders = 1u;
        n_waves = 16u;
    }
    if (n_slots < 2u * n_loaders || n_slots > 8u) n_slots = 8u;
    if (n_waves < 8u || n_waves > 16u) n_waves = 8u;
    if (!claim.ctr || !uniform_n || uniform_n % 2048u) return false;
    const uint32_t ntiles = ring_tiles(ratio, ntaps, uniform_n);
    if (!ring_limits_ok(ntiles, claim, ratio >= 32)) return false;
    if ((ratio <= 4) != (final_call != nullptr)) return false;
    RingArgs ra{in, in_stride, hist_in, hist_out, taps, out, out_stride, uniform_n, ntiles, claim, gave_up, final_call, fir_hist_cap, fft_in};
#define HD_S1_CASE(D, T)                                                                                                              \
    if (ratio == D && ntaps == T) {                                                                                                   \
        static_assert(D >= 32 || (uint32_t)ring_bytes<T, kRingNSLAlone>() <= 163840u, "eight tile slots must fit a CU's LDS");       \
        const uint32_t workers = D == 32 ? 8u : n_slots <= 4u ? 3u : 4u;             \
        const uint32_t lds = D >= 32 ? workers * (uint32_t)work_slot_bytes<(D >= 32 ? D : 32)>() : n_slots * (uint32_t)ring_slot_bytes<T>() + (uint32_t)kRingCtlBytes; \
        static bool attr_set[64] = {};                                                                                                \
        int dev_ = 0;                                                                                                                 \
        if (hipGetDevice(&dev_) != hipSuccess || dev_ < 0 || dev_ >= 64) return false;                                                \
        if (!attr_set[dev_]) {                                                                                                        \
            if (hipFuncSetAttribute(reinterpret_cast<const void*>(k_stage1_cu<T, D>), hipFuncAttributeMaxDynamicSharedMemorySize, 163840) != hipSuccess) return false; \
            attr_set[dev_] = true;                                                                                                    \
        }                                                                                                                             \
        hipLaunchKernelGGL((k_stage1_cu<T, D>), dim3(n_cus), dim3(64u * (D == 4 ? n_waves : D >= 32 ? workers : 8u)), lds, st, ra, n_loaders, n_slots);   \
        return true;                                                                                                                  \
    }
    HD_S1_CASE(32, 212) HD_S1_CASE(32, 174) HD_S1_CASE(64, 348) HD_S1_CASE(8, 54) HD_S1_CASE(4, 139)
#undef HD_S1_CASE
    return false;
}

uint32_t probe_xcc_mask(hipStream_t st, uint32_t n_cus, unsigned int* d_word)
{
    if (hipMemsetAsync(d_word, 0, 4, st) != hipSuccess) return 0;
    hipLaunchKernelGGL(k_xcc_probe, dim3(n_cus * 8u), dim3(64), 0, st, d_word);
    unsigned int h = 0;
    if (hipMemcpyAsync(&h, d_word, 4, hipMemcpyDeviceToHost, st) != hipSuccess || hipStreamSynchronize(st) != hipSuccess) return 0;
    return h;
}

void launch_passthrough(hipStream_t st, uint32_t n_streams, uint32_t max_n, const float2* in, size_t in_stride, float2* out,
                        size_t out_stride, const StreamCall* call, uint32_t fir_hist_cap)
{
    if (!max_n) return;
    dim3 grid((max_n + 255) / 256, n_streams);
    hipLaunchKernelGGL(k_passthrough, grid, dim3(256), 0, st, in, in_stride, out, out_stride, call, fir_hist_cap);
}

void launch_chunk_post(hipStream_t st, uint32_t n_streams, float2* fbuf, size_t stride, const StreamCall* call, uint32_t fir_hist_cap,
                       const uint2* tune, const float* tune_tab)
{
    hipLaunchKernelGGL(k_dc_remove, dim3(n_streams), dim3(64), 0, st, fbuf, stride, call, fir_hist_cap, tune, tune_tab);
}

}
}
```

habdec_amd/csrc/kernels/launch.h:

```cpp
#pragma once
#include <hip/hip_runtime.h>
#include <stddef.h>
#include <stdint.h>

#include "../dev_types.h"

namespace hd {

struct DemodCarry {
    float re, im;
    uint32_t primed;
    uint32_t _pad;
};

struct StepClaim {
    unsigned int* ctr = nullptr;
    unsigned int* ctr_next = nullptr;
    uint32_t n_xcd = 0, runs_per_xcd = 0, run_len = 0;
    uint32_t short_from = 0xFFFFFFFFu, tiles_per_xcd = 0;
};

struct TailArgs {
    const float2* dec1; size_t dec1_stride;
    const float2* hist2_in; float2* hist2_out; const float* taps2;
    float2* fbuf; float2* fbuf_next; size_t fbuf_stride; uint32_t fir_hist_cap;
    const float* lp_taps; uint32_t taps_stride;
    float* demod; size_t demod_stride; float2* filtered;
    const DemodCarry* carry_in; DemodCarry* carry_out;
    const StreamCall* call; float2* fft_in;
    float2* head_buf ; const float2* fbuf_prev ; uint32_t head_cap, n_streams;
    float* ring; uint32_t ring_cap; SymState* sym; unsigned long long* flipmask; float* wsum; const SymbolParams* sp;
    uint32_t* slots; uint32_t slot_words; uint32_t* flips_dbg; uint32_t flips_cap;
    uint32_t seq;
    const float2* fft_tw; float2* spec; float* power; SpectrumStatsDev* stats; double rate; int bins_sep;
    uint32_t pend_max, f_off, v_off, ws_off, words_off, tp_off, h2_off, flips_off, fl_cap, strips_off, dyn_off, lds_bytes;
    uint32_t op;
    const uint2* tune; const float* tune_tab;
};

constexpr uint32_t kStepLdsBytes = 20480;

void launch_spectrum_wave(hipStream_t st, uint32_t n_streams, const float2* fft_in, const float2* tw4096, float2* spec, float* power,
                          SpectrumStatsDev* stats, const StreamCall* call, double rate, int bins_sep,
                          uint32_t seq ,
                          const float2* chunk = nullptr ,
                          size_t chunk_stride = 0, uint32_t fir_hist_cap = 0);

namespace exact {
#include "launch_decls.inc"
}
namespace fast {
#include "launch_decls.inc"
}

}
```

habdec_amd/csrc/kernels/launch_decls.inc:

```
bool launch_decimate(hipStream_t st, int ratio, int ntaps, uint32_t n_streams, uint32_t max_out,
                     const float2* in, size_t in_stride, const float2* hist_in, float2* hist_out, const float* taps,
                     float2* out, size_t out_stride, const StreamCall* call, int stage, int final_stage,
                     uint32_t fir_hist_cap, float2* fft_in ,
                     uint32_t lin_wgs = 0 ,
                     StreamCall* call_copy = nullptr ,
                     uint32_t uniform_n = 0 ,
                     const StepClaim& claim = StepClaim{} );
bool launch_decimate_tuned(hipStream_t st, int ratio, int ntaps, uint32_t n_streams, uint32_t max_out,
                           const float2* in, size_t in_stride, const float2* hist_in, float2* hist_out, const float* taps,
                           float2* out, size_t out_stride, const StreamCall* call, int final_stage,
                           uint32_t fir_hist_cap, float2* fft_in, uint32_t lin_wgs, const uint2* ftune, const float* ftab);
void launch_fetch_params(hipStream_t st, const void* host_mapped, void* dst, size_t bytes);
void launch_passthrough(hipStream_t st, uint32_t n_streams, uint32_t max_n, const float2* in, size_t in_stride,
                        float2* out, size_t out_stride, const StreamCall* call, uint32_t fir_hist_cap);
void launch_chunk_post(hipStream_t st, uint32_t n_streams, float2* fbuf, size_t stride, const StreamCall* call, uint32_t fir_hist_cap,
                       const uint2* tune, const float* tune_tab);
void launch_fft_feed(hipStream_t st, uint32_t n_streams, const float2* fbuf, size_t stride, float2* fft_in,
                     const StreamCall* call, uint32_t fir_hist_cap);
void launch_fir_demod(hipStream_t st, uint32_t n_streams, uint32_t max_m, uint32_t max_taps, const float2* fbuf, size_t stride,
                      const float* taps, uint32_t taps_stride, float* demod, size_t demod_stride, float2* filtered ,
                      const DemodCarry* carry_in, DemodCarry* carry_out, const StreamCall* call, uint32_t fir_hist_cap,
                      float* sym_ring, uint32_t ring_cap, const SymState* sym, float2* fbuf_next,
                      float2* head_side , uint32_t head_cap, const float2* fbuf_prev ,
                      uint32_t* ck_acc = nullptr ,
                      const float2* pre = nullptr ,
                      uint32_t pre_stride = 0, float pre_scale = 1.0f);
void launch_lp_gather(hipStream_t st, uint32_t n_streams, const float2* fbuf, size_t stride, float2* work, uint32_t N, const StreamCall* call, uint32_t fir_hist_cap,
                      const float2* head_side, uint32_t head_cap, const float2* fbuf_prev);
void launch_lp_taps_gather(hipStream_t st, uint32_t n_streams, const float* taps, uint32_t taps_stride, const uint32_t* ntaps, float2* kf, uint32_t N);
void launch_lp_mul(hipStream_t st, uint32_t n_streams, float2* work, const float2* kf, uint32_t N, const StreamCall* call);
bool tail_layout(TailArgs& a, int lanes, int ratio2, int ntaps2, uint32_t max_taps, uint32_t max_R, uint32_t min_R, uint32_t ring_cap,
                 uint32_t pend_max , uint32_t lds_limit,
                 int op = 0 );
bool launch_tail(hipStream_t st, int lanes, int ratio2, int ntaps2, uint32_t n_streams, const TailArgs& a, hipEvent_t ev_stop = nullptr);
bool launch_step(hipStream_t st, int ratio, int ntaps, int ratio2, int ntaps2, uint32_t n_streams, uint32_t n_out, const float2* in, size_t in_stride,
                 const float2* hist_in, float2* hist_out, const float* taps, float2* out, size_t out_stride, const StreamCall* call,
                 StreamCall* call_copy, uint32_t stage1_wgs, const TailArgs& ta, uint32_t n_tail,
                 uint32_t uniform_n ,
                 const StepClaim& claim = StepClaim{});
bool launch_step_cu(hipStream_t st, int ratio, int ntaps, int ratio2, int ntaps2, uint32_t n_streams, uint32_t n_cus, const float2* in, size_t in_stride,
                    const float2* hist_in, float2* hist_out, const float* taps, float2* out, size_t out_stride, const StreamCall* call,
                    StreamCall* call_copy, const TailArgs& ta, uint32_t n_tail, uint32_t uniform_n, const StepClaim& claim, uint32_t tail_bytes,
                    hipEvent_t ev_start = nullptr, hipEvent_t ev_stop = nullptr );
uint32_t ring_tiles(int ratio, int ntaps, uint32_t n);
bool step_cu_supported(int ratio, int ntaps, int ratio2, int ntaps2);
bool stage1_cu_supported(int ratio, int ntaps);
bool launch_stage1_cu(hipStream_t st, int ratio, int ntaps, uint32_t n_cus, const float2* in, size_t in_stride, const float2* hist_in, float2* hist_out,
                      const float* taps, float2* out, size_t out_stride, uint32_t uniform_n, const StepClaim& claim, unsigned int* gave_up,
                      uint32_t n_loaders , uint32_t n_waves ,
                      uint32_t n_slots = 8 ,
                      const StreamCall* final_call = nullptr ,
                      uint32_t fir_hist_cap = 0, float2* fft_in = nullptr);
uint32_t step_cu_tail_lds(int ratio, int ntaps);
uint32_t probe_xcc_mask(hipStream_t st, uint32_t n_cus, unsigned int* d_word);
uint32_t step_lds_bytes(int ratio, int ntaps);
void launch_symbols(hipStream_t st, uint32_t n_streams, uint32_t max_m, uint32_t max_new, uint32_t max_R, const float* tail,
                    uint32_t ring_cap, SymState* sym, unsigned long long* flipmask, float* weight, const SymbolParams* sp,
                    const StreamCall* call, uint32_t* slots, uint32_t slot_words, uint32_t* flips_dbg, uint32_t flips_cap,
                    uint32_t min_R ,
                    uint32_t seq ,
                    hipEvent_t ev_stop = nullptr ,
                    uint32_t* ck_acc = nullptr );
```

habdec_amd/csrc/kernels/stage1_ring.h:

```cpp
#pragma once
#include <hip/hip_runtime.h>

#include "arith.h"
#include "launch.h"

namespace hd {
namespace HD_ARITH_NS {

typedef float r_f32x2 __attribute__((ext_vector_type(2)));
typedef float r_f32x4 __attribute__((ext_vector_type(4)));

constexpr int kRingRowBytes = 272;
constexpr int kRingNSLAlone = 4;
constexpr int kWorkSlotBytes = 64 * kRingRowBytes;
constexpr int kRingCtlBytes = 384;
constexpr uint32_t kRingSpinLimit = 1u << 22;
template <int T> constexpr int ring_halo_rows() { return (T - 1 + 31) / 32; }
template <int T> constexpr int ring_slot_bytes() { return (64 + ring_halo_rows<T>()) * kRingRowBytes; }
template <int T, int NSL = kRingNSLAlone> constexpr int ring_bytes() { return 2 * NSL * ring_slot_bytes<T>() + kRingCtlBytes; }
template <int T> constexpr int ring_adv() { return 64 - ring_halo_rows<T>(); }

__host__ __device__ constexpr uint32_t ring_sys_tiles(uint32_t n, uint32_t adv) { return (n / 32u + adv - 1u) / adv; }

#ifdef HD_STAMP_RING
__device__ unsigned long long g_ring_stamps[512 * 8 * 8];
extern "C" void HD_DBG_NAME(hd_debug_ring_stamps)(unsigned long long* host, size_t n) { (void)hipMemcpyFromSymbol(host, HIP_SYMBOL(g_ring_stamps), n * 8); }
#define RSTAMP_DECL unsigned long long rs_t = __builtin_amdgcn_s_memtime(), rs_acc[6] = {0, 0, 0, 0, 0, 0}; const unsigned long long rs_r0 = __builtin_amdgcn_s_memrealtime()
#define RSTAMP(i) do { const unsigned long long t_ = __builtin_amdgcn_s_memtime(); rs_acc[i] += t_ - rs_t; rs_t = t_; } while (0)
#define RSTAMP_WRITE(wave_, n_) do { if ((threadIdx.x & 63u) == 0 && blockIdx.x < 512 && (wave_) < 8u) { unsigned long long* g_ = g_ring_stamps + ((size_t)blockIdx.x * 8 + (wave_)) * 8; \
        for (int i_ = 0; i_ < 5; ++i_) g_[i_] = rs_acc[i_]; g_[5] = (n_); g_[6] = rs_r0; g_[7] = __builtin_amdgcn_s_memrealtime(); } } while (0)
#else
#define RSTAMP_DECL do { } while (0)
#define RSTAMP(i) do { } while (0)
#define RSTAMP_WRITE(wave_, n_) do { } while (0)
#endif

#ifdef HD_RING_FAULT
__device__ unsigned int g_ring_fault_fired, g_ring_fault_mode;
static void ring_fault_arm(unsigned int mode) { const unsigned int z = 0; (void)hipMemcpyToSymbol(HIP_SYMBOL(g_ring_fault_mode), &mode, sizeof mode); (void)hipMemcpyToSymbol(HIP_SYMBOL(g_ring_fault_fired), &z, sizeof z); }
extern "C" void HD_DBG_NAME(hd_debug_ring_fault_arm)() { ring_fault_arm(0u); }
extern "C" void HD_DBG_NAME(hd_debug_ring_fault_arm_starve)() { ring_fault_arm(1u); }
#endif

constexpr uint32_t kSlotFree = 0u, kSlotReady = 1u, kSlotTaken = 2u;
struct RingCtl {
    unsigned long long slot[16];
    uint32_t live;
    uint32_t run_tail;
    uint32_t run_head;
    uint32_t _pad0;
    uint32_t run_q[4];
    uint32_t simd_rank[4];
    uint32_t roles_taken;
    uint32_t _pad[3];
};
static_assert(sizeof(RingCtl) <= kRingCtlBytes, "ring control block");
__device__ __forceinline__ void ring_ctl_init(RingCtl* ctl, const uint32_t n_live)
{
    const uint32_t i = threadIdx.x;
    if (i < (uint32_t)kRingCtlBytes / 4u) reinterpret_cast<uint32_t*>(ctl)[i] = i == (uint32_t)offsetof(RingCtl, live) / 4u ? n_live : 0u;
}

struct RingGeom {
    unsigned char* ring; uint32_t nb;
};

struct RingArgs {
    const float2* in; size_t in_stride;
    const float2* hist_in; float2* hist_out;
    const float* taps;
    float2* out; size_t out_stride;
    uint32_t n;
    uint32_t ntiles;
    StepClaim claim;
    unsigned int* gave_up;
    const StreamCall* call; uint32_t fir_hist_cap; float2* fft_in;
};

__device__ __forceinline__ uint32_t lds_addr_of(const void* p)
{
    return (uint32_t)(uintptr_t)(const __attribute__((address_space(3))) void*)p;
}

__device__ __forceinline__ void wait_vmcnt(uint32_t n)
{
#define HD_VMC(k) case k: asm volatile("s_waitcnt vmcnt(" #k ")" ::: "memory"); break;
    switch (n) {
        HD_VMC(0) HD_VMC(1) HD_VMC(2) HD_VMC(3) HD_VMC(4) HD_VMC(5) HD_VMC(6) HD_VMC(7) HD_VMC(8) HD_VMC(9)
        HD_VMC(10) HD_VMC(11) HD_VMC(12) HD_VMC(13) HD_VMC(14) HD_VMC(15) HD_VMC(16) HD_VMC(17) HD_VMC(18) HD_VMC(19)
        HD_VMC(20) HD_VMC(21) HD_VMC(22) HD_VMC(23) HD_VMC(24) HD_VMC(25) HD_VMC(26) HD_VMC(27) HD_VMC(28) HD_VMC(29)
        HD_VMC(30) HD_VMC(31) HD_VMC(32) HD_VMC(33) HD_VMC(34) HD_VMC(35) HD_VMC(36) HD_VMC(37) HD_VMC(38) HD_VMC(39)
        HD_VMC(40) HD_VMC(41) HD_VMC(42) HD_VMC(43) HD_VMC(44) HD_VMC(45) HD_VMC(46) HD_VMC(47) HD_VMC(48) HD_VMC(49)
        HD_VMC(50) HD_VMC(51) HD_VMC(52) HD_VMC(53) HD_VMC(54) HD_VMC(55) HD_VMC(56) HD_VMC(57) HD_VMC(58) HD_VMC(59)
        HD_VMC(60) HD_VMC(61) HD_VMC(62)
        default: asm volatile("s_waitcnt vmcnt(63)" ::: "memory"); break;
    }
#undef HD_VMC
}

__device__ __forceinline__ void glds16(const void* base, uint32_t off, uint32_t lds_dst)
{
    unsigned keep;
    asm volatile("s_mov_b32 %0, m0\n\ts_mov_b32 m0, %3\n\ts_nop 0\n\tglobal_load_lds_dwordx4 %1, %2\n\ts_mov_b32 m0, %0"
                 : "=&s"(keep) : "v"(off), "s"(base), "s"(lds_dst) : "memory");
}
__device__ __forceinline__ void glds4(const void* base, uint32_t off, uint32_t lds_dst)
{
    unsigned keep;
    asm volatile("s_mov_b32 %0, m0\n\ts_mov_b32 m0, %3\n\ts_nop 0\n\tglobal_load_lds_dword %1, %2\n\ts_mov_b32 m0, %0"
                 : "=&s"(keep) : "v"(off), "s"(base), "s"(lds_dst) : "memory");
}

template <bool HEAD_KEPT = false >
__device__ __forceinline__ void glds16_x17(const void* base, const uint32_t (&off)[17], uint32_t lds_dst)
{
    unsigned keep, scc_keep;
#define HD_GLDS_BODY_POLICY " nt"
#define HD_G1(n) "global_load_lds_dwordx4 %" #n ", %19" HD_GLDS_BODY_POLICY "\n\ts_add_u32 m0, m0, 0x400\n\ts_nop 0\n\t"
#define HD_G1D(n) "global_load_lds_dwordx4 %" #n ", %19\n\ts_add_u32 m0, m0, 0x400\n\ts_nop 0\n\t"
#define HD_G17_OPS : "=&s"(keep), "=&s"(scc_keep)                                                                                                                   \
                   : "v"(off[0]), "v"(off[1]), "v"(off[2]), "v"(off[3]), "v"(off[4]), "v"(off[5]), "v"(off[6]), "v"(off[7]), "v"(off[8]), "v"(off[9]),              \
                     "v"(off[10]), "v"(off[11]), "v"(off[12]), "v"(off[13]), "v"(off[14]), "v"(off[15]), "v"(off[16]), "s"(base), "s"(lds_dst)                      \
                   : "memory"
    if constexpr (HEAD_KEPT)
        asm volatile("s_cselect_b32 %1, 1, 0\n\ts_mov_b32 %0, m0\n\ts_mov_b32 m0, %20\n\ts_nop 0\n\t"
                     HD_G1D(2) HD_G1D(3) HD_G1(4) HD_G1(5) HD_G1(6) HD_G1(7) HD_G1(8) HD_G1(9) HD_G1(10) HD_G1(11) HD_G1(12) HD_G1(13) HD_G1(14) HD_G1(15) HD_G1(16) HD_G1D(17)
                     "global_load_lds_dwordx4 %18, %19\n\ts_mov_b32 m0, %0\n\ts_cmp_lg_u32 %1, 0" HD_G17_OPS);
    else
        asm volatile("s_cselect_b32 %1, 1, 0\n\ts_mov_b32 %0, m0\n\ts_mov_b32 m0, %20\n\ts_nop 0\n\t"
                     HD_G1(2) HD_G1(3) HD_G1(4) HD_G1(5) HD_G1(6) HD_G1(7) HD_G1(8) HD_G1(9) HD_G1(10) HD_G1(11) HD_G1(12) HD_G1(13) HD_G1(14) HD_G1(15) HD_G1(16) HD_G1D(17)
                     "global_load_lds_dwordx4 %18, %19\n\ts_mov_b32 m0, %0\n\ts_cmp_lg_u32 %1, 0" HD_G17_OPS);
#undef HD_G17_OPS
#undef HD_G1D
// ... 483 lines not shown
template <int T, int D = 32>
__device__ __forceinline__ void ring_worker(const RingArgs& a, unsigned char* __restrict__ slot, const uint32_t role )
{
    static_assert(D == 32 || D == 64, "a row is one output's stride");
    constexpr int HR = work_halo_rows<T, D>();
    constexpr uint32_t ADV = 64u - (uint32_t)HR;
    constexpr int JS = HR * D - (T - 1);
    constexpr int NS = JS + T;
    constexpr int CPR = D / 2 + 1;
    constexpr int ROWB = work_row_bytes<D>();
    constexpr int NX = D / 2;
    constexpr int UPS = D / 32;
    constexpr int NU = (HR + 1) * UPS;
    constexpr int NB0 = ((int)ADV * CPR + 63) / 64;
    constexpr int HQ = D / 32;
    static_assert(NS == HR * D + 1, "the window ends with slot 0 of row HR");
    const uint32_t lane = threadIdx.x & 63u;
    typedef const float __attribute__((address_space(4)))* ctaps_t;
    const ctaps_t taps = (ctaps_t)(uintptr_t)a.taps - JS;
    const uint32_t dst = (uint32_t)__builtin_amdgcn_readfirstlane((int)lds_addr_of(slot));
    const unsigned char* p = slot + lane * (uint32_t)ROWB;
    const uint32_t rows = a.n / (uint32_t)D;
    RSTAMP_DECL;
    uint32_t n_done = 0; (void)n_done;

    uint32_t boff[CPR], hist_off[HR * HQ];
#pragma unroll
    for (int i = 0; i < CPR; ++i) { const uint32_t P = 64u * i + lane, row = P / (uint32_t)CPR, col = P - row * (uint32_t)CPR; boff[i] = row * (uint32_t)(D * 8) + (col < (uint32_t)(CPR - 1) ? col : (uint32_t)(CPR - 2)) * 16u; }
#pragma unroll
    for (int r = 0; r < HR * HQ; ++r) {
        const int h = (r / HQ - HR) * D + (r % HQ) * 32 + (int)(lane >> 1) + (T - 1);
        hist_off[r] = (uint32_t)(h < 0 ? 0 : h) * 8u + (lane & 1u) * 4u;
    }
    auto issue = [&](const uint32_t s, const uint32_t tile, const bool run_start) {
        const unsigned char* in_s = reinterpret_cast<const unsigned char*>(a.in + (size_t)s * a.in_stride);
        if (tile == 0) {
            const unsigned char* hb = reinterpret_cast<const unsigned char*>(a.hist_in + (size_t)s * (T - 1));
#pragma unroll
            for (int r = 0; r < HR * HQ; ++r) glds4(hb, hist_off[r], dst + (uint32_t)((r / HQ) * ROWB + (r % HQ) * 256));
#pragma unroll
            for (int i = 0; i < NB0; ++i)
                if (64 * (i + 1) <= (int)ADV * CPR || lane < (uint32_t)((int)ADV * CPR - 64 * i)) glds16(in_s, boff[i], dst + (uint32_t)(HR * ROWB) + 1024u * i);
        } else {
            const uint32_t origin = tile * ADV < rows - ADV ? tile * ADV : rows - ADV;
            const unsigned char* src = in_s + (size_t)(origin - (uint32_t)HR) * (uint32_t)(D * 8);
            if constexpr (D == 32) { if (run_start) glds16_x17<true>(src, boff, dst); else glds16_x17<false>(src, boff, dst); }
            else { glds16_x11<11>(src, boff, dst); glds16_x11<11>(src, boff + 11, dst + 11u * 1024u); glds16_x11<7>(src, boff + 22, dst + 22u * 1024u); }
        }
    };

    const uint32_t xcd0 = __builtin_amdgcn_s_getreg((3 << 11) | (0 << 6) | 20) & 15u;
    const uint32_t xcd = xcd0 < a.claim.n_xcd ? xcd0 : a.claim.n_xcd - 1;
    unsigned int* my_ctr = a.claim.ctr + (size_t)xcd * 32;
    unsigned int* next_ctr = a.claim.ctr_next + (size_t)xcd * 32;
    const uint32_t runs = a.claim.runs_per_xcd, run_len = a.claim.run_len, short_from = a.claim.short_from < runs ? a.claim.short_from : runs;
    const uint32_t tpx = a.claim.tiles_per_xcd ? a.claim.tiles_per_xcd : runs * run_len;
    auto draw = [&]() -> unsigned int { unsigned int t = 0; if (lane == 0) t = __hip_atomic_fetch_add(my_ctr, 1u, __ATOMIC_RELAXED, __HIP_MEMORY_SCOPE_AGENT); return t; };
    uint32_t s = 0, tile = 0, left = 0, this_run = 0;
    auto take_run = [&](const unsigned int ticket) -> bool {
        const uint32_t t = (uint32_t)__builtin_amdgcn_readfirstlane((int)ticket);
        if (t == runs && lane == 0) (void)__hip_atomic_exchange(next_ctr, 0u, __ATOMIC_RELAXED, __HIP_MEMORY_SCOPE_AGENT);
        if (t >= runs) return false;
        const uint32_t g0 = xcd * tpx + (t < short_from ? t * run_len : short_from * run_len + (t - short_from));
        s = g0 / a.ntiles; tile = g0 - s * a.ntiles; left = this_run = t < short_from ? run_len : 1u;
        return true;
    };
    auto advance = [&]() { ++tile; --left; if (tile == a.ntiles) { tile = 0; ++s; } };

    asm volatile("s_waitcnt lgkmcnt(0)" ::: "memory");
    if (!take_run(draw())) { RSTAMP_WRITE(role, 0); return; }
    uint32_t cs = s, ct = tile;
    issue(cs, ct, true); advance();
    unsigned int ticket = 0;
    if (!left) ticket = draw();

    auto ldk = [&](r_f32x2 (&k)[8], auto cc) {
        constexpr int c = decltype(cc)::value;
#pragma unroll
        for (int j = 0; j < 16; j += 2) {
            k[j >> 1].x = (16 * c + j >= JS && 16 * c + j < NS) ? taps[16 * c + j] : 0.f;
            k[j >> 1].y = (16 * c + j + 1 >= JS && 16 * c + j + 1 < NS) ? taps[16 * c + j + 1] : 0.f;
        }
    };
    for (;;) {
        RSTAMP(2);
        asm volatile("s_waitcnt vmcnt(0)" ::: "memory");
        asm volatile("" : "+v"(ticket));
        RSTAMP(0);
        r_f32x2 kk[2][2][8];
        r_f32x4 x[NX];
#pragma unroll
        for (int q = 0; q < NX; ++q) x[q] = *reinterpret_cast<const r_f32x4*>(p + 16 * q);
        ldk(kk[0][0], std::integral_constant<int, 0>{}); ldk(kk[0][1], std::integral_constant<int, 1>{});
        __builtin_amdgcn_sched_barrier(0);
#pragma unroll
        for (int q = 0; q < NX; q += 8)
            asm volatile("" : "+v"(x[q]), "+v"(x[q + 1]), "+v"(x[q + 2]), "+v"(x[q + 3]), "+v"(x[q + 4]), "+v"(x[q + 5]), "+v"(x[q + 6]), "+v"(x[q + 7]) :: "memory");
        RSTAMP(3);
        bool more = true;
        if (!left) more = take_run(ticket);
        uint32_t ns = 0, nt = 0;
        if (more) {
            ns = s; nt = tile;
            issue(ns, nt, left == this_run); advance();
            if (!left) ticket = draw();
        }
        RSTAMP(4);

        const uint32_t origin = ct * ADV < rows - ADV ? ct * ADV : rows - ADV;
        r_f32x2 acc = {0.f, 0.f};
#ifdef HD_FAST_ARITH
        r_f32x2 acc_b = {0.f, 0.f};
#endif
        auto mac_chunk = [&](const r_f32x2 (&k)[8], auto cc) {
            constexpr int c = decltype(cc)::value, j0 = JS > 16 * c ? JS - 16 * c : 0, j1 = NS < 16 * c + 16 ? NS - 16 * c : 16;
            const r_f32x4 (&xh)[8] = reinterpret_cast<const r_f32x4 (&)[8]>(x[8 * (c % (D / 16))]);
#ifdef HD_FAST_ARITH
            if constexpr (j0 == 0 && j1 == 16) ring_fma16x2(acc, acc_b, xh, k);
            else {
#pragma unroll
                for (int j = j0; j < j1; ++j) {
                    const r_f32x2 smp = (j & 1) ? xh[j >> 1].zw : xh[j >> 1].xy;
                    const float kj = (j & 1) ? k[j >> 1].y : k[j >> 1].x;
                    if (j & 1) acc_b = __builtin_elementwise_fma(smp, (r_f32x2){kj, kj}, acc_b);
                    else acc = __builtin_elementwise_fma(smp, (r_f32x2){kj, kj}, acc);
                }
            }
#else
            if constexpr (j0 == 0 && j1 == 16) ring_mac16_asm(acc, xh, k);
            else {
#pragma unroll
                for (int j = j0; j < j1; ++j) {
                    const r_f32x2 smp = (j & 1) ? xh[j >> 1].zw : xh[j >> 1].xy;
                    acc = acc + smp * ((j & 1) ? k[j >> 1].y : k[j >> 1].x);
                }
            }
#endif
        };
        auto rot1 = [&](r_f32x2& v) {
            const float re = v.x, im = v.y;
            v.x = __builtin_bit_cast(float, __builtin_amdgcn_update_dpp(0, __builtin_bit_cast(int, re), 0x13C, 0xF, 0xF, false));
            v.y = __builtin_bit_cast(float, __builtin_amdgcn_update_dpp(0, __builtin_bit_cast(int, im), 0x13C, 0xF, 0xF, false));
        };
        auto rot = [&]() {
            rot1(acc);
#ifdef HD_FAST_ARITH
            rot1(acc_b);
#endif
        };
        auto arrived = [&](const r_f32x2 (&k)[2][8]) {
            asm volatile("" :: "s"(k[0][0]), "s"(k[0][1]), "s"(k[0][2]), "s"(k[0][3]), "s"(k[0][4]), "s"(k[0][5]), "s"(k[0][6]), "s"(k[0][7]),
                               "s"(k[1][0]), "s"(k[1][1]), "s"(k[1][2]), "s"(k[1][3]), "s"(k[1][4]), "s"(k[1][5]), "s"(k[1][6]), "s"(k[1][7]));
        };
        ring_for_each_index([&](auto ui) {
            constexpr int u = decltype(ui)::value;
            arrived(kk[u & 1]);
            if constexpr (u + 1 < NU) {
                ldk(kk[(u + 1) & 1][0], std::integral_constant<int, 2 * u + 2>{});
                ldk(kk[(u + 1) & 1][1], std::integral_constant<int, 2 * u + 3>{});
            }
            __builtin_amdgcn_sched_barrier(0);
            if constexpr (JS < 32 * u + 16 && 32 * u < NS) mac_chunk(kk[u & 1][0], std::integral_constant<int, 2 * u>{});
            if constexpr (32 * u + 16 < NS && JS < 32 * u + 32) mac_chunk(kk[u & 1][1], std::integral_constant<int, 2 * u + 1>{});
            if constexpr ((u + 1) % UPS == 0 && u + 1 < NU) rot();
        }, std::make_integer_sequence<int, NU>{});
#ifdef HD_FAST_ARITH
        acc = acc + acc_b;
#endif
#ifdef HD_STAMP_RING
        asm volatile("" : "+v"(acc));
        ++n_done;
#endif
        RSTAMP(1);
        if (lane >= (uint32_t)HR) a.out[(size_t)cs * a.out_stride + origin + lane - (uint32_t)HR] = make_float2(acc.x, acc.y);
        if (ct + 1 == a.ntiles) {
            const float2* in_s = a.in + (size_t)cs * a.in_stride + (a.n - (uint32_t)(T - 1));
            float2* hout = a.hist_out + (size_t)cs * (T - 1);
            constexpr int NH = (T - 1 + 63) / 64;
            float2 h[NH];
#pragma unroll
            for (int k = 0; k < NH; ++k) h[k] = in_s[lane + 64u * k < (uint32_t)(T - 1) ? lane + 64u * k : 0u];
#pragma unroll
            for (int k = 0; k < NH; ++k) if (lane + 64u * k < (uint32_t)(T - 1)) hout[lane + 64u * k] = h[k];
        }
        if (!more) break;
        cs = ns; ct = nt;
    }
    RSTAMP(2);
    RSTAMP_WRITE(role, n_done);
}

}
}
```

habdec_amd/csrc/kernels/tail_body.h:

```cpp
#pragma once
#include <hip/hip_runtime.h>

#include "arith.h"
#include "exact_math.h"
#include "launch.h"
#include "sym_common.h"
#include "spectrum_wave.h"
#include "tune.h"

namespace hd {
namespace HD_ARITH_NS {

constexpr uint32_t kTailHdrBytes = 64;
constexpr uint32_t kTailStrip = 512;

typedef float f32x4 __attribute__((ext_vector_type(4)));
typedef const float __attribute__((address_space(4)))* cfloat_ptr;
__device__ __forceinline__ cfloat_ptr as_const(const float* p) { return (cfloat_ptr)(uintptr_t)p; }

#define HD_TB_TAP4(A_, B_, C_, D_, k_)                                                        \
    {                                                                                         \
        HD_FIR_ARITH                                                                          \
        const f32x2 p0_ = (A_) * (k_), p1_ = (B_) * (k_), p2_ = (C_) * (k_), p3_ = (D_) * (k_); \
        a0 = a0 + p0_; a1 = a1 + p1_; a2 = a2 + p2_; a3 = a3 + p3_;                           \
// ... 348 lines not shown
            for (int q = 0; q < OP; ++q) {
                const uint32_t th = tn.y + (o0 + OP * tid + q) * tn.x;
                const float2 cc = tab2[th >> 24], ff = tab2[kTuneTable + ((th >> 16) & 255u)];
                tpc[q] = make_float4(cc.x, cc.y, ff.x, ff.y);
            }
        }
#pragma unroll
        for (int u = 0; u < XB; ++u) {
            *reinterpret_cast<float4*>(X + xp0 + u * kXStepP) = tx[u];
        }
        tb_sync<NT>();
        if (pc + 1 < npieces) prefetch(pc + 1);
        TSTAMP(2);

        {
            constexpr int NWIN = ((D2 * (OP - 1) + 3) >> 1) + 1;
            const f32x4* h2 = reinterpret_cast<const f32x4*>(H2);
            const f32x4* px = reinterpret_cast<const f32x4*>(X + xpos((uint32_t)(OP * tid) * D2));
            f32x4 kc = h2[0];
            f32x2 acc[OP];
            f32x4 win[NWIN];
#pragma unroll
            for (int q = 0; q < OP; ++q) acc[q] = (f32x2){0.f, 0.f};
            constexpr int NB4 = T2 / 4;
            auto block = [&](const f32x4 n0, const f32x4 n1, const f32x4 kn) {
                __builtin_amdgcn_sched_barrier(0);
                tb_s2_tap<0, OP, D2, NWIN>(acc, win, kc.x);
                tb_s2_tap<1, OP, D2, NWIN>(acc, win, kc.y);
                tb_s2_tap<2, OP, D2, NWIN>(acc, win, kc.z);
                tb_s2_tap<3, OP, D2, NWIN>(acc, win, kc.w);
#pragma unroll
                for (int j = 0; j + 2 < NWIN; ++j) win[j] = win[j + 2];
                win[NWIN - 2] = n0; win[NWIN - 1] = n1;
                kc = kn;
            };
            if constexpr (kXPad) {
                static_assert(NWIN == 5, "the padded image's offsets below are those of four outputs per lane at /2");
#pragma unroll
                for (int j = 0; j < NWIN; ++j) win[j] = px[j + (j >> 2)];
                const f32x4* pq = px;
                int b = 0;
#pragma unroll 1
                for (; b + 2 <= NB4; b += 2, pq += 5) {
                    { const f32x4 n0 = pq[6], n1 = pq[7]; const f32x4 kn = h2[b + 1]; block(n0, n1, kn); }
                    { const f32x4 n0 = pq[8], n1 = pq[10]; const f32x4 kn = h2[b + 2]; block(n0, n1, kn); }
                }
                if (b < NB4) { const f32x4 n0 = pq[6], n1 = pq[7]; const f32x4 kn = h2[b + 1]; block(n0, n1, kn); }
            } else {
#pragma unroll
                for (int j = 0; j < NWIN; ++j) win[j] = px[j];
#pragma unroll 2
                for (int b = 0; b < NB4; ++b) {
                    const f32x4 n0 = px[2 * b + NWIN], n1 = px[2 * b + NWIN + 1];
                    const f32x4 kn = h2[b + 1];
                    block(n0, n1, kn);
                }
            }
            if constexpr (T2 % 4 >= 1) tb_s2_tap<0, OP, D2, NWIN>(acc, win, kc.x);
            if constexpr (T2 % 4 >= 2) tb_s2_tap<1, OP, D2, NWIN>(acc, win, kc.y);
            if constexpr (T2 % 4 >= 3) tb_s2_tap<2, OP, D2, NWIN>(acc, win, kc.z);
            TSTAMP(18);
            const bool keepF = keepf || npieces == 1;
            if (rot) {
                const uint32_t q4_lo = n1 - (uint32_t)(T2 - 1);
#pragma unroll
                for (int q = 0; q < OP; ++q) {
                    const uint32_t ol = OP * tid + q, oo = o0 + ol;
                    if (pc + 1 == npieces && n1 && ol < po && oo >= q4_lo && oo < n2)
                        a.hist2_out[(size_t)s * (T2 - 1) + (oo - q4_lo)] = make_float2(acc[q].x, acc[q].y);
                    float yr, yi;
                    tune_apply(tpc[q].x, tpc[q].y, tpc[q].z, tpc[q].w, acc[q].x, acc[q].y, yr, yi);
                    acc[q] = (f32x2){yr, yi};
                }
            }
            bool done4 = false;
            if constexpr (OP == 4) {
                const uint32_t oo = o0 + 4 * tid;
                if (4 * tid + 3 < po && !(pb & 1u)) {
                    const float4 y01 = make_float4(acc[0].x, acc[0].y, acc[1].x, acc[1].y), y23 = make_float4(acc[2].x, acc[2].y, acc[3].x, acc[3].y);
                    if (keepF) { float4* f4 = reinterpret_cast<float4*>(F + (f_old + oo - fbase)); f4[0] = y01; f4[1] = y23; }
                    { float4* c4 = reinterpret_cast<float4*>(cur + fhc + pb + oo); c4[0] = y01; c4[1] = y23; }
                    if (a.fft_in && oo < c.fft_take) {
                        float2* fi = a.fft_in + (size_t)s * kFftBins + c.fft_fill + oo;
                        if (oo + 3 < c.fft_take && !(c.fft_fill & 1u)) { reinterpret_cast<float4*>(fi)[0] = y01; reinterpret_cast<float4*>(fi)[1] = y23; }
                        else {
#pragma unroll
                            for (int q = 0; q < 4; ++q) if (oo + q < c.fft_take) fi[q] = make_float2(acc[q].x, acc[q].y);
                        }
                    }
                    done4 = true;
                }
            }
            if (!done4) {
#pragma unroll
                for (int q = 0; q < OP; ++q) {
                    const uint32_t ol = OP * tid + q;
                    if (ol < po) {
                        const uint32_t oo = o0 + ol;
                        const float2 y = make_float2(acc[q].x, acc[q].y);
                        if (keepF) F[f_old + oo - fbase] = y;
                        cur[fhc + pb + oo] = y;
                        if (a.fft_in && oo < c.fft_take) a.fft_in[(size_t)s * kFftBins + c.fft_fill + oo] = y;
                    }
                }
            }
        }
        float2 xt[HB];
#pragma unroll
        for (int u = 0; u < HB; ++u) { const uint32_t k = tid + u * NT; xt[u] = k < (uint32_t)(T2 - 1) ? X[xh0 + kXPiece + u * kXStepH] : make_float2(0.f, 0.f); }
        if (pc + 1 == npieces && n1) {
            tb_sync<NT>();
            for (uint32_t k = tid; k < (uint32_t)(T2 - 1); k += NT) {
                const uint32_t idx = n1 - (T2 - 1) + k;
                if (rot && idx < n2) continue;
                a.hist2_out[(size_t)s * (T2 - 1) + k] = idx < n2 ? F[f_old + idx - fbase] : in_s[idx];
            }
        }
        tb_sync<NT>();
#pragma unroll
        for (int u = 0; u < HB; ++u) { const uint32_t k = tid + u * NT; if (k < (uint32_t)(T2 - 1)) X[xh0 + u * kXStepH] = xt[u]; }
        fcount += po;
        TSTAMP(3);

        if (run && ((pc & 1u) || pc + 1 == npieces)) {
            const uint32_t i_hi = (pc + 1 == npieces) ? m : min(m, (pb + o0 + po) & ~1u);
            const f32x4* hk = reinterpret_cast<const f32x4*>(TP);
            float2* Yl = Y;
            if (kCompact) { if (tid == 0) Yl[0] = carryY[0]; }
            const uint32_t c0v = c0;
            for (uint32_t i0 = i_done; i0 < i_hi; i0 += 8 * NT) {
                const uint32_t live = min((uint32_t)(8 * NT), i_hi - i0);
                const uint32_t nvA = 4u * tid < live ? min(4u, live - 4u * tid) : 0u;
                const uint32_t nvB = 4u * NT + 4u * tid < live ? min(4u, live - 4u * NT - 4u * tid) : 0u;
                f32x2 a0 = {0.f, 0.f}, a1 = {0.f, 0.f}, a2 = {0.f, 0.f}, a3 = {0.f, 0.f};
                f32x2 b0 = {0.f, 0.f}, b1 = {0.f, 0.f}, b2 = {0.f, 0.f}, b3 = {0.f, 0.f};
                {
                    const f32x4* pA = reinterpret_cast<const f32x4*>(F + (i0 - fbase)) + 2 * tid;
                    const f32x4* pB = live > 4u * NT ? pA + 2 * NT : pA;
                    f32x4 A0 = pA[0], A1 = pA[1], A2 = pA[2], A3 = pA[3], A4, A5;
                    f32x4 B0 = pB[0], B1 = pB[1], B2 = pB[2], B3 = pB[3], B4, B5;
                    f32x4 kc = hk[0], k1, k2;
                    uint32_t t = 0;
                    for (; t + 12 <= T; t += 12) {
                        const uint32_t j = t >> 1, jk = t >> 2;
                        A4 = pA[j + 4]; A5 = pA[j + 5]; B4 = pB[j + 4]; B5 = pB[j + 5]; k1 = hk[jk + 1];
                        __builtin_amdgcn_sched_barrier(0);
                        HD_TB_BLK(A0, A1, A2, A3, kc, a0, a1, a2, a3)
                        HD_TB_BLK(B0, B1, B2, B3, kc, b0, b1, b2, b3)
                        A0 = pA[j + 6]; A1 = pA[j + 7]; B0 = pB[j + 6]; B1 = pB[j + 7]; k2 = hk[jk + 2];
                        __builtin_amdgcn_sched_barrier(0);
                        HD_TB_BLK(A2, A3, A4, A5, k1, a0, a1, a2, a3)
                        HD_TB_BLK(B2, B3, B4, B5, k1, b0, b1, b2, b3)
                        A2 = pA[j + 8]; A3 = pA[j + 9]; B2 = pB[j + 8]; B3 = pB[j + 9]; kc = hk[jk + 3];
                        __builtin_amdgcn_sched_barrier(0);
                        HD_TB_BLK(A4, A5, A0, A1, k2, a0, a1, a2, a3)
                        HD_TB_BLK(B4, B5, B0, B1, k2, b0, b1, b2, b3)
                    }
                    for (; t + 4 <= T; t += 4) {
                        const uint32_t j = t >> 1;
                        A4 = pA[j + 4]; A5 = pA[j + 5]; B4 = pB[j + 4]; B5 = pB[j + 5]; k1 = hk[(t >> 2) + 1];
                        HD_TB_BLK(A0, A1, A2, A3, kc, a0, a1, a2, a3)
                        HD_TB_BLK(B0, B1, B2, B3, kc, b0, b1, b2, b3)
                        A0 = A2; A1 = A3; A2 = A4; A3 = A5; B0 = B2; B1 = B3; B2 = B4; B3 = B5; kc = k1;
                    }
                    if (t < T) { HD_TB_TAPN(A0.xy, A0.zw, A1.xy, A1.zw, kc.x, a0, a1, a2, a3) HD_TB_TAPN(B0.xy, B0.zw, B1.xy, B1.zw, kc.x, b0, b1, b2, b3) ++t; }
                    if (t < T) { HD_TB_TAPN(A0.zw, A1.xy, A1.zw, A2.xy, kc.y, a0, a1, a2, a3) HD_TB_TAPN(B0.zw, B1.xy, B1.zw, B2.xy, kc.y, b0, b1, b2, b3) ++t; }
                    if (t < T) { HD_TB_TAPN(A1.xy, A1.zw, A2.xy, A2.zw, kc.z, a0, a1, a2, a3) HD_TB_TAPN(B1.xy, B1.zw, B2.xy, B2.zw, kc.z, b0, b1, b2, b3) ++t; }
                    const f32x2 lastA = nvA == 4 ? a3 : nvA == 3 ? a2 : nvA == 2 ? a1 : a0;
                    const f32x2 lastB = nvB == 4 ? b3 : nvB == 3 ? b2 : nvB == 2 ? b1 : b0;
                    Yl[1 + tid] = make_float2(lastA.x, lastA.y);
                    Yl[1 + NT + tid] = make_float2(lastB.x, lastB.y);
                }
                TSTAMP(12);
                tb_sync<NT>();
                {
                    f32x2 c0 = a0, c1 = a1, c2 = a2, c3 = a3;
                    uint32_t nv = nvA, i = i0 + 4 * tid;
                    float2 qv = Yl[tid];
#pragma unroll 1
                    for (int w = 0; w < 2; ++w) {
                        if (nv) {
                            float pr = qv.x, pi = qv.y;
                            if (i == 0 && !kin.primed) { pr = c0.x; pi = c0.y; }
                            float d[4];
                            d[0] = discriminate(c0.x, c0.y, pr, pi);
                            d[1] = discriminate(c1.x, c1.y, c0.x, c0.y);
                            d[2] = discriminate(c2.x, c2.y, c1.x, c1.y);
                            d[3] = discriminate(c3.x, c3.y, c2.x, c2.y);
                            const f32x2 av[4] = {c0, c1, c2, c3};
#pragma unroll
                            for (int u = 0; u < 4; ++u)
                                if ((uint32_t)u < nv) { const uint32_t b = __builtin_bit_cast(uint32_t, d[u]); ck0 += b; ck1 += (i + (uint32_t)u + 1u) * b; }
                            float* dm = a.demod + (size_t)s * a.demod_stride + i;
                            const uint32_t pos = end_old + i;
                            const float4 d4 = make_float4(d[0], d[1], d[2], d[3]);
                            if (nv == 4 && !(i & 3u)) *reinterpret_cast<float4*>(dm) = d4;
                            else {
                                if (nv >= 2) *reinterpret_cast<float2*>(dm) = make_float2(d[0], d[1]); else dm[0] = d[0];
                                if (nv == 4) *reinterpret_cast<float2*>(dm + 2) = make_float2(d[2], d[3]); else if (nv == 3) dm[2] = d[2];
                            }
                            if (nv == 4 && !(pos & 3u)) *reinterpret_cast<float4*>(vring + (pos & rmask)) = d4;
                            else {
#pragma unroll
                                for (int u = 0; u < 4; ++u) if ((uint32_t)u < nv) vring[(pos + u) & rmask] = d[u];
                            }
                            if (do_sums) {
                                if (nv == 4 && !((pos - c0v) & 3u)) *reinterpret_cast<float4*>(V + (pos - c0v)) = d4;
                                else {
#pragma unroll
                                    for (int u = 0; u < 4; ++u) if ((uint32_t)u < nv) V[pos + u - c0v] = d[u];
                                }
                            }
                            if (a.filtered) {
#pragma unroll
                                for (int u = 0; u < 4; ++u) if ((uint32_t)u < nv) a.filtered[(size_t)s * a.demod_stride + i + u] = make_float2(av[u].x, av[u].y);
                            }
                            if (i + nv == m) {
                                DemodCarry k; k.primed = 1; k._pad = 0;
                                const f32x2 lastv = nv == 4 ? c3 : nv == 3 ? c2 : nv == 2 ? c1 : c0;
                                k.re = lastv.x; k.im = lastv.y;
                                a.carry_out[s] = k;
                            }
                        }
                        c0 = b0; c1 = b1; c2 = b2; c3 = b3; nv = nvB; i = i0 + 4 * NT + 4 * tid; qv = Yl[NT + tid];
                    }
                }
                TSTAMP(14);
                tb_sync<NT>();
                {
                    const uint32_t lo = live - 1, lw = lo / (4u * NT), ll = (lo % (4u * NT)) >> 2;
                    if (tid == ll) { const float2 cy = Yl[1 + lw * NT + tid]; Yl[0] = cy; if (kCompact) carryY[0] = cy; }
                }
            }
            i_done = i_hi;
            TSTAMP(4);
            {
                const uint32_t shf = i_done - fbase, keep = fcount - shf;
                if (shf) {
                    tb_sync<NT>();
                    for (uint32_t k0 = 0; k0 < keep; k0 += 4 * NT) {
                        float2 t4[4];
#pragma unroll
                        for (int u = 0; u < 4; ++u) { const uint32_t k = k0 + tid + u * NT; t4[u] = k < keep ? F[k + shf] : make_float2(0.f, 0.f); }
                        tb_sync<NT>();
#pragma unroll
                        for (int u = 0; u < 4; ++u) { const uint32_t k = k0 + tid + u * NT; if (k < keep) F[k] = t4[u]; }
                    }
                    fbase = i_done; fcount = keep;
                }
            }
            TSTAMP(5);
            if (do_sums) vcnt = end_old + i_done - c0;
        }
        ++pc;
    }
    tb_sync<NT>();

    const uint32_t h = st.held;
    const uint32_t end = st.base + h;
    const uint32_t pend = end - R + 1;
    const bool hunt = m && do_sums && search;
    const uint32_t limit = hunt ? h - q.spb : 0u;
    const uint32_t carried_to = st.run_pos - st.base;
    const uint32_t wr0 = (st.base + R) & ~63u;
    const uint32_t nw = hunt ? ((st.base + limit) - wr0 + 63u) >> 6 : 0u;
    const uint32_t lmw = (nw + 1u) & ~1u;
    const uint32_t dyn_floats = hunt ? (((a.lds_bytes - a.dyn_off) - lmw * 8u) >> 2) & ~3u : 0u;
    const uint32_t vc_want = (hunt && limit > carried_to) ? limit - carried_to : 0u;
    const uint32_t woff = st.base & 3u, voff = (st.base + carried_to) & 3u;
    const uint32_t vc_cap = min((vc_want + voff + 7u) & ~3u, (dyn_floats * 5u / 8u) & ~3u);
    const uint32_t wc_cap = dyn_floats - vc_cap;
    const uint32_t wc_n = hunt ? min(limit, wc_cap > woff + 4u ? wc_cap - woff - 4u : 0u) : 0u;
    const uint32_t vc_n = min(vc_want, vc_cap > voff + 4u ? vc_cap - voff - 4u : 0u);
    const uint32_t wq_n = wc_n ? (wc_n + woff + 3u) >> 2 : 0u, vq_n = vc_n ? (vc_n + voff + 3u) >> 2 : 0u;
    const uint32_t wpos4 = st.base & ~3u, vpos4 = (st.base + carried_to) & ~3u;
    constexpr int MB = 512 / NT, CB = 1024 / NT / 4 > 0 ? 1024 / NT / 4 : 1, SB = CB;
    unsigned long long tm0[MB];
    float4 tc0[CB], ts0[SB];
    if (hunt) {
        __threadfence_block();
#pragma unroll
        for (int u = 0; u < MB; ++u) { const uint32_t i = tid + u * NT; tm0[u] = i < nw ? gmask[((wr0 + 64u * i) & rmask) >> 6] : 0ull; }
// ... 264 lines not shown
```

include/habdec_amd_host.h:

```cpp
#ifndef HABDEC_AMD_HOST_H
#define HABDEC_AMD_HOST_H
#include <stddef.h>
#include <stdint.h>
#ifdef __cplusplus
extern "C" {
#endif

int hd_host_decim_plan(unsigned total_factor, int ratio[2], unsigned ntaps[2]);
size_t hd_host_decim_taps(unsigned total_factor, int stage, float* taps, size_t cap);

size_t hd_host_lowpass_design(float cutoff_rel, float transition, size_t batch, size_t prev_ntaps, int float_trig,
                              float* taps, size_t cap);

typedef struct hd_host_rtty hd_host_rtty;
hd_host_rtty* hd_host_rtty_new(size_t nbits, float nstops);
void hd_host_rtty_free(hd_host_rtty*);
size_t hd_host_rtty_push_run(hd_host_rtty*, const uint8_t* bits, size_t n, char* out, size_t cap);
size_t hd_host_rtty_pending(const hd_host_rtty*);

void hd_host_crc16(const char* s, size_t n, char out4[5]);
int hd_host_extract_sentence(const char* stream, size_t n, char* callsign, char* data, char* crc, char* rest, size_t cap);

typedef struct hd_host_text hd_host_text;
hd_host_text* hd_host_text_new(size_t nbits, float nstops);
void hd_host_text_free(hd_host_text*);
void hd_host_text_push_bits(hd_host_text*, const uint8_t* bits, size_t n);
size_t hd_host_text_get(hd_host_text*, int which , char* buf, size_t cap);

typedef struct hd_host_afc hd_host_afc;
hd_host_afc* hd_host_afc_new(void);
void hd_host_afc_free(hd_host_afc*);
void hd_host_afc_step(hd_host_afc*, int have_spectrum, int valid, int peak1, int peak2, float power1, float power2,
                      double mean, double sigma, size_t bins, double rate);
void hd_host_afc_reset(hd_host_afc*, double correction, size_t bins, double rate);
void hd_host_afc_get(hd_host_afc*, double* correction, double* shift_hz, double* noise_floor, double* noise_sigma,
                     int* peak_l, int* peak_r);

void hd_host_atan2f(const float* y, const float* x, float* out, size_t n);
void hd_host_discriminate(const float* iq, size_t n, float prev_re, float prev_im, float* out);

size_t hd_host_spectrum_payload(const float* bins, size_t n, double noise_floor, double noise_variance, double sampling_rate, double shift,
                                int peak_left, int peak_right, float zoom, int resolution, int type_size, uint8_t* out, size_t cap,
                                size_t* bins_sent);
size_t hd_host_demod_payload(const float* trace, size_t n, int resolution, int type_size, uint8_t* out, size_t cap, size_t* values_sent);

typedef struct hd_host_telemetry {
    char callsign[64];
    int32_t frame, hour, minute;
    float second, lat, lon, alt;
} hd_host_telemetry;
int hd_host_parse_time(const char* text, int* hour, int* minute, float* second);
int hd_host_parse_gps_pos(const char* text, float* out);
int hd_host_parse_sentence(const char* sentence_without_crc, hd_host_telemetry* out);
size_t hd_host_timestamp_from_hms(int64_t now_unix, int hour, int minute, float second, char* buf, size_t cap);
void hd_host_gps_distance(double lat1, double lon1, double alt1, double lat2, double lon2, double alt2, double out[5]);

typedef struct hd_host_sondehub hd_host_sondehub;
hd_host_sondehub* hd_host_sondehub_new(const char* uploader_callsign, const char* software_version );
void hd_host_sondehub_free(hd_host_sondehub*);
int hd_host_sondehub_push_sentence(hd_host_sondehub*, uint32_t stream, const char* callsign, const char* data, int64_t now_unix_ns);
int hd_host_sondehub_push(hd_host_sondehub*, const char* payload_callsign, const char* time_received, const char* datetime, int frame,
                          float lat, float lon, float alt);
size_t hd_host_sondehub_size(const hd_host_sondehub*);
size_t hd_host_sondehub_take(hd_host_sondehub*, int64_t now_unix_ns, char* out, size_t cap, size_t* n_records);
size_t hd_host_utc_iso(int64_t unix_ns, char* buf, size_t cap);
size_t hd_host_json_number(double v, char* buf, size_t cap);

typedef struct hd_host_iqfiles hd_host_iqfiles;
hd_host_iqfiles* hd_host_iqfiles_open(const char* const* paths, uint32_t n_files, int loop, uint32_t chunk, uint32_t granule,
                                      double realtime_rate);
void hd_host_iqfiles_close(hd_host_iqfiles*);
uint32_t hd_host_iqfiles_streams(const hd_host_iqfiles*);
uint64_t hd_host_iqfiles_count(const hd_host_iqfiles*, uint32_t stream);
uint64_t hd_host_iqfiles_rewinds(const hd_host_iqfiles*, uint32_t stream);
uint32_t hd_host_iqfiles_next(hd_host_iqfiles*, float* slab, size_t stride, uint32_t* n_per_stream);

int  hd_host_tune_step(double offset_hz, double decimated_rate, uint32_t* step);
void hd_host_tune_tables(float coarse[512], float fine[512]);
void hd_host_tune_rotate(const float* iq, size_t n, uint32_t phase, uint32_t step, float* out);

#ifdef __cplusplus
}
#endif
#endif
```

Measured before the change: 495,300.

## Time step kernel with in-kernel wall clock and use write-through streaming stores

Timed step launches now record per-block wall_clock64 first-start and last-end into a device record that is copied to pinned host memory, instead of wrapping the launch in HIP events. The stage-1 ring worker writes outputs with a buffer store carrying a cache-policy bit and waits only on older stores (vmcnt(1)) rather than draining its own last store. Tail-stage FFT-input and demod outputs go through sc1/agent-scope atomic stores. These changes aim to cut event overhead on timed calls and to reduce cache pollution and store-wait stalls, at the cost of extra atomics per block and a host spin-wait on the clock tag.

Result: no change. 503,700, median of 6 (+1.7%).

```diff
diff --git a/habdec_amd/capi.py b/habdec_amd/capi.py
--- a/habdec_amd/capi.py
+++ b/habdec_amd/capi.py
@@ -146,6 +146,7 @@
     "hd_host_tune_step": (_int, [_dbl, _dbl, C.POINTER(C.c_uint32)]),
     "hd_host_tune_tables": (None, [_f32p, _f32p]),
     "hd_host_tune_rotate": (None, [_f32p, _sz, C.c_uint32, C.c_uint32, _f32p]),
+    "hd_host_step_clock_ms": (_dbl, [C.c_uint64, C.c_uint32]),
 }
 
 
diff --git a/habdec_amd/csrc/dev_types.h b/habdec_amd/csrc/dev_types.h
--- a/habdec_amd/csrc/dev_types.h
+++ b/habdec_amd/csrc/dev_types.h
@@ -69,6 +69,16 @@
 };
 static_assert(sizeof(BitsHeader) == 48, "result slot header");
 
+struct StepClockRec {
+    unsigned long long first_start, last_end;
+    uint32_t arrived, _pad;
+};
+struct StepClockOut {
+    unsigned long long first_start, last_end;
+    uint32_t seq, _pad;
+};
+inline double step_clock_ms(unsigned long long ticks, uint32_t rate_khz) { return rate_khz ? (double)ticks / (double)rate_khz : 0.0; }
+
 struct SpectrumStatsDev {
     int32_t valid;
     int32_t peak1, peak2;
diff --git a/habdec_amd/csrc/engine.cpp b/habdec_amd/csrc/engine.cpp
--- a/habdec_amd/csrc/engine.cpp
+++ b/habdec_amd/csrc/engine.cpp
@@ -150,6 +150,8 @@
     bool device_failed = false;
     uint64_t step_launches = 0;
     DevBuf<unsigned int> step_ctr;
+    DevBuf<hd::StepClockRec> step_clock;
+    uint32_t wall_khz = 0;
     uint32_t pend_max_taps = 0;
     bool dec_wgs_forced = false;
 #ifdef HD_TIMING_EXPERIMENT
@@ -198,6 +200,8 @@
         PinBuf<uint2> h_tune;
         PinBuf<uint2> h_front;
         bool timed = false, timed_step = false;
+        bool clocked = false;
+        PinBuf<hd::StepClockOut> h_clock;
         hipEvent_t ev_front = nullptr, ev_done = nullptr, ev_params = nullptr, ev_spec = nullptr, t0 = nullptr, t1 = nullptr, t2 = nullptr, t3 = nullptr;
         bool busy = false;
         uint32_t seq = 0;
@@ -388,6 +392,16 @@
     if (e->stages.size() == 2) for (auto* b : {&e->dec1, &e->dec1b, &e->dec1c}) HD_HIP(b->alloc((size_t)S * e->n1_cap));
     HD_HIP(e->step_ctr.alloc(2 * 16 * 32 + 32));
     HD_HIP(e->ring_gave_up.alloc(4));
+    {
+        HD_HIP(e->step_clock.alloc(hd_engine::kSlots));
+        hd::StepClockRec idle[hd_engine::kSlots];
+        for (auto& r : idle) r = hd::StepClockRec{~0ull, 0ull, 0u, 0u};
+        HD_HIP(hipMemcpy(e->step_clock.p, idle, sizeof idle, hipMemcpyHostToDevice));
+        for (auto& sl : e->slot) HD_HIP(sl.h_clock.alloc(1));
+        int khz = 0;
+        HD_HIP(hipDeviceGetAttribute(&khz, hipDeviceAttributeWallClockRate, cfg->device));
+        e->wall_khz = khz > 0 ? (uint32_t)khz : 0u;
+    }
     e->ring_gave_up.p[0] = 0;
     if (!e->no_claim && e->n_cus % 32u == 0) {
         const uint32_t n_xcd = e->n_cus / 32u;
@@ -692,7 +706,21 @@
     sl.busy = false;
     if (sl.timed) {
         float a = 0, b = 0;
-        HD_HIP(hipEventElapsedTime(&b, sl.t1, sl.t2));
+        if (sl.clocked) {
+            const volatile hd::StepClockOut* ck = sl.h_clock.p;
+            const auto t_lim = std::chrono::steady_clock::now() + std::chrono::milliseconds(200);
+            for (uint32_t spins = 0; ck->seq != sl.seq; ++spins) {
+                if (std::chrono::steady_clock::now() > t_lim) {
+                    e->device_failed = true;
+                    e->fail_cause = "the step launch's clock block does not carry its call's tag 200 ms after the completion event";
+                    break;
+                }
+                if (spins > 64u) std::this_thread::yield();
+            }
+            std::atomic_thread_fence(std::memory_order_acquire);
+            const unsigned long long t_first = ck->first_start, t_last = ck->last_end;
+            b = e->device_failed || t_last < t_first ? 0.f : (float)hd::step_clock_ms(t_last - t_first, e->wall_khz);
+        } else { HD_HIP(hipEventElapsedTime(&b, sl.t1, sl.t2)); }
         if (sl.timed_step) a = b; else HD_HIP(hipEventElapsedTime(&a, sl.t0, sl.t3));
         e->last_timing.ms_total = a;
         e->last_timing.ms_front = b;
@@ -1017,6 +1045,7 @@
     if (!r.lean && !r.free_front && e->calls >= 2 && !e->one_stream) HD_HIP(hipStreamWaitEvent(qa, e->slot[(e->calls - 2) % hd_engine::kSlots].ev_done, 0));
     const bool step = r.route == Route::step;
     sl.timed = e->timing_every && (e->calls % e->timing_every) == 0;
+    sl.clocked = false;
     sl.timed_step = sl.timed && step;
     if (sl.timed && !step) HD_HIP(hipEventRecord(sl.t0, qa));
     if (!r.lean && !r.free_front && !r.host_params) {
@@ -1075,8 +1104,10 @@
         launched = HDK(launch_step_cu, qa, R1, T1, prev.valid ? prev.r2 : R2, prev.valid ? prev.t2 : T2, S, e->n_cus, iq, stride,
                                       e->hist1[b.hin].p, e->hist1[b.hout].p, e->stage_taps[0].p, b.d1, e->n1_cap, sl.h_call.dev, sl.d_call.p, prev.ta,
                                       (prev.valid && !(cu_exp & 1)) ? S : 0u, p.max_in, cl, tb,
-                                      sl.timed ? sl.t1 : nullptr, sl.timed ? sl.t2 : ps ? ps->ev_done : nullptr);
-    }
+                                      (sl.timed && !hd::kStepKernelClock) ? sl.t1 : nullptr, (sl.timed && !hd::kStepKernelClock) ? sl.t2 : ps ? ps->ev_done : nullptr,
+                                      (sl.timed && hd::kStepKernelClock) ? hd::StepClock{e->step_clock.p + (&sl - e->slot), sl.h_clock.dev, sl.seq} : hd::StepClock{});
+    }
+    sl.clocked = launched && sl.timed && hd::kStepKernelClock;
     e->last_timing.step_variant = launched ? 1u : 0u;
     if (launched) ++e->step_launches;
     else {
@@ -1094,7 +1125,7 @@
         if (fb.ctr) ++e->step_launches;
     }
     if (sl.timed && !launched) HD_HIP(hipEventRecord(sl.t2, qa));
-    if (ps && (!launched || sl.timed)) HD_HIP(hipEventRecord(ps->ev_done, qa));
+    if (ps && (!launched || (sl.timed && !hd::kStepKernelClock))) HD_HIP(hipEventRecord(ps->ev_done, qa));
     HD_HIP(hipGetLastError());
     return HD_OK;
 }
diff --git a/habdec_amd/csrc/host_api.cpp b/habdec_amd/csrc/host_api.cpp
--- a/habdec_amd/csrc/host_api.cpp
+++ b/habdec_amd/csrc/host_api.cpp
@@ -13,6 +13,7 @@
 #include "host/iq_file_batch.hpp"
 #include "host/tune_host.hpp"
 #include "kernels/exact_math.h"
+#include "dev_types.h"
 
 struct hd_host_rtty { hd::RttyFramer f; };
 struct hd_host_text { hd::TextStage t; };
@@ -246,6 +247,7 @@
     return 0;
 }
 void hd_host_tune_tables(float coarse[512], float fine[512]) { hd::tune_tables(coarse, fine); }
+double hd_host_step_clock_ms(uint64_t ticks, uint32_t rate_khz) { return hd::step_clock_ms(ticks, rate_khz); }
 void hd_host_tune_rotate(const float* iq, size_t n, uint32_t phase, uint32_t step, float* out)
 {
     float tab[4 * hd::kTuneTable];
diff --git a/habdec_amd/csrc/kernels/decimate.hip b/habdec_amd/csrc/kernels/decimate.hip
--- a/habdec_amd/csrc/kernels/decimate.hip
+++ b/habdec_amd/csrc/kernels/decimate.hip
@@ -542,14 +542,37 @@
                             blockIdx.x - n_tail, 0u, gridDim.x - n_tail, tile4, uniform_n, claim);
 }
 
+__device__ __forceinline__ void step_clock_leave(RingCtl* ctl, const StepClock& clk)
+{
+    asm volatile("s_waitcnt vmcnt(0)" ::: "memory");
+    const uint32_t lane = threadIdx.x & 63u;
+    uint32_t gone = 0;
+    if (lane == 0) gone = __hip_atomic_fetch_add(&ctl->gone, 1u, __ATOMIC_ACQ_REL, __HIP_MEMORY_SCOPE_WORKGROUP);
+    if ((uint32_t)__builtin_amdgcn_readfirstlane((int)gone) + 1u != blockDim.x / 64u) return;
+    if (lane != 0) return;
+    (void)__hip_atomic_fetch_max(&clk.rec->last_end, (unsigned long long)wall_clock64(), __ATOMIC_RELAXED, __HIP_MEMORY_SCOPE_AGENT);
+    asm volatile("s_waitcnt vmcnt(0)" ::: "memory");
+    const uint32_t before = __hip_atomic_fetch_add(&clk.rec->arrived, 1u, __ATOMIC_RELAXED, __HIP_MEMORY_SCOPE_AGENT);
+    if (before + 1u != gridDim.x) return;
+    const unsigned long long t_first = __hip_atomic_exchange(&clk.rec->first_start, ~0ull, __ATOMIC_RELAXED, __HIP_MEMORY_SCOPE_AGENT);
+    const unsigned long long t_last = __hip_atomic_exchange(&clk.rec->last_end, 0ull, __ATOMIC_RELAXED, __HIP_MEMORY_SCOPE_AGENT);
+    (void)__hip_atomic_exchange(&clk.rec->arrived, 0u, __ATOMIC_RELAXED, __HIP_MEMORY_SCOPE_AGENT);
+    __hip_atomic_store(&clk.out->first_start, t_first, __ATOMIC_RELAXED, __HIP_MEMORY_SCOPE_SYSTEM);
+    __hip_atomic_store(&clk.out->last_end, t_last, __ATOMIC_RELAXED, __HIP_MEMORY_SCOPE_SYSTEM);
+    asm volatile("s_waitcnt vmcnt(0)" ::: "memory");
+    __hip_atomic_store(&clk.out->seq, clk.seq, __ATOMIC_RELAXED, __HIP_MEMORY_SCOPE_SYSTEM);
+}
+
 template <int T, int D2, int T2>
 __global__ __launch_bounds__(512) void k_step_cu(const RingArgs ra, const StreamCall* __restrict__ call, StreamCall* __restrict__ call_copy,
-                                                 const TailArgs ta, const uint32_t n_tail, const uint32_t n_streams, const uint32_t tail_bytes )
+                                                 const TailArgs ta, const uint32_t n_tail, const uint32_t n_streams, const uint32_t tail_bytes ,
+                                                 const StepClock clk)
 {
     extern __shared__ __attribute__((aligned(16))) unsigned char cu_lds[];
     RingCtl* ctl = reinterpret_cast<RingCtl*>(cu_lds);
     unsigned char* slots = cu_lds + kRingCtlBytes;
     unsigned char* tails = slots + 4 * kWorkSlotBytes;
+    if (clk.rec && threadIdx.x == 0) (void)__hip_atomic_fetch_min(&clk.rec->first_start, (unsigned long long)wall_clock64(), __ATOMIC_RELAXED, __HIP_MEMORY_SCOPE_AGENT);
     ring_ctl_init(ctl, 0u);
     __syncthreads();
     const uint32_t simd = (__builtin_amdgcn_s_getreg((2 - 1) << 11 | 4 << 6 | 4)) & 3u;
@@ -585,6 +608,7 @@
         }
         ring_worker<T>(ra, n_tail ? tails + k * tail_bytes : slots + w * (uint32_t)kWorkSlotBytes, w);
     }
+    if (clk.rec) step_clock_leave(ctl, clk);
 }
 
 template <int T, int D>
@@ -780,7 +804,7 @@
 bool launch_step_cu(hipStream_t st, int ratio, int ntaps, int ratio2, int ntaps2, uint32_t n_streams, uint32_t n_cus, const float2* in, size_t in_stride,
                     const float2* hist_in, float2* hist_out, const float* taps, float2* out, size_t out_stride, const StreamCall* call,
                     StreamCall* call_copy, const TailArgs& ta, uint32_t n_tail, uint32_t uniform_n, const StepClaim& claim, uint32_t tail_bytes,
-                    hipEvent_t ev_start, hipEvent_t ev_stop)
+                    hipEvent_t ev_start, hipEvent_t ev_stop, const StepClock& clock)
 {
     if (ratio != 32 || !claim.ctr || !uniform_n || uniform_n % 2048u) return false;
     const uint32_t ntiles = ring_tiles(ratio, ntaps, uniform_n);
@@ -801,8 +825,8 @@
         }                                                                                                                             \
         const dim3 grid_(n_cus > (n_streams + 3u) / 4u ? n_cus : (n_streams + 3u) / 4u);                                             \
              \
-        if (ev_start || ev_stop) hipExtLaunchKernelGGL((k_step_cu<T, D2, T2>), grid_, dim3(512), lds, st, ev_start, ev_stop, 0u, ra, call, call_copy, ta, n_tail, n_streams, tail_bytes); \
-        else hipLaunchKernelGGL((k_step_cu<T, D2, T2>), grid_, dim3(512), lds, st, ra, call, call_copy, ta, n_tail, n_streams, tail_bytes); \
+        if (ev_start || ev_stop) hipExtLaunchKernelGGL((k_step_cu<T, D2, T2>), grid_, dim3(512), lds, st, ev_start, ev_stop, 0u, ra, call, call_copy, ta, n_tail, n_streams, tail_bytes, clock); \
+        else hipLaunchKernelGGL((k_step_cu<T, D2, T2>), grid_, dim3(512), lds, st, ra, call, call_copy, ta, n_tail, n_streams, tail_bytes, clock); \
         return true;                                                                                                                  \
     }
     HD_CU_CASE(212, 2, 69) HD_CU_CASE(174, 4, 139)
diff --git a/habdec_amd/csrc/kernels/launch.h b/habdec_amd/csrc/kernels/launch.h
--- a/habdec_amd/csrc/kernels/launch.h
+++ b/habdec_amd/csrc/kernels/launch.h
@@ -18,6 +18,45 @@
     unsigned int* ctr_next = nullptr;
     uint32_t n_xcd = 0, runs_per_xcd = 0, run_len = 0;
     uint32_t short_from = 0xFFFFFFFFu, tiles_per_xcd = 0;
+};
+
+#if defined(HD_TIMING_EXPERIMENT) && defined(HD_EXP_EVENT_CLOCK)
+constexpr bool kStepKernelClock = false;
+#else
+constexpr bool kStepKernelClock = true;
+#endif
+#if defined(HD_TIMING_EXPERIMENT) && defined(HD_EXP_NO_WT_STAGE1)
+constexpr bool kWtStage1 = false;
+#else
+constexpr bool kWtStage1 = true;
+#endif
+#if defined(HD_TIMING_EXPERIMENT) && defined(HD_EXP_NO_WT_TAIL)
+constexpr bool kWtTail = false;
+#else
+constexpr bool kWtTail = true;
+#endif
+#if defined(HD_TIMING_EXPERIMENT) && defined(HD_EXP_WAIT_OWN_STORE)
+constexpr bool kWorkerWaitsOwnStore = true;
+#else
+constexpr bool kWorkerWaitsOwnStore = false;
+#endif
+
+template <bool WT, class V> __device__ __forceinline__ void store_once(V* p, const V v)
+{
+    static_assert(sizeof(V) == 4 || sizeof(V) == 8 || sizeof(V) == 16, "a dword, a pair or a quad");
+    if constexpr (!WT) *p = v;
+    else if constexpr (sizeof(V) == 4) __hip_atomic_store(reinterpret_cast<uint32_t*>(p), __builtin_bit_cast(uint32_t, v), __ATOMIC_RELAXED, __HIP_MEMORY_SCOPE_AGENT);
+    else if constexpr (sizeof(V) == 8) __hip_atomic_store(reinterpret_cast<unsigned long long*>(p), __builtin_bit_cast(unsigned long long, v), __ATOMIC_RELAXED, __HIP_MEMORY_SCOPE_AGENT);
+    else {
+        typedef float q_f32x4 __attribute__((ext_vector_type(4)));
+        asm volatile("global_store_dwordx4 %0, %1, off sc1\n\ts_nop 1" :: "v"(p), "v"(__builtin_bit_cast(q_f32x4, v)) : "memory");
+    }
+}
+
+struct StepClock {
+    StepClockRec* rec = nullptr;
+    StepClockOut* out = nullptr;
+    uint32_t seq = 0;
 };
 
 struct TailArgs {
diff --git a/habdec_amd/csrc/kernels/launch_decls.inc b/habdec_amd/csrc/kernels/launch_decls.inc
--- a/habdec_amd/csrc/kernels/launch_decls.inc
+++ b/habdec_amd/csrc/kernels/launch_decls.inc
@@ -41,7 +41,8 @@
 bool launch_step_cu(hipStream_t st, int ratio, int ntaps, int ratio2, int ntaps2, uint32_t n_streams, uint32_t n_cus, const float2* in, size_t in_stride,
                     const float2* hist_in, float2* hist_out, const float* taps, float2* out, size_t out_stride, const StreamCall* call,
                     StreamCall* call_copy, const TailArgs& ta, uint32_t n_tail, uint32_t uniform_n, const StepClaim& claim, uint32_t tail_bytes,
-                    hipEvent_t ev_start = nullptr, hipEvent_t ev_stop = nullptr );
+                    hipEvent_t ev_start = nullptr, hipEvent_t ev_stop = nullptr ,
+                    const StepClock& clock = StepClock{} );
 uint32_t ring_tiles(int ratio, int ntaps, uint32_t n);
 bool step_cu_supported(int ratio, int ntaps, int ratio2, int ntaps2);
 bool stage1_cu_supported(int ratio, int ntaps);
diff --git a/habdec_amd/csrc/kernels/stage1_ring.h b/habdec_amd/csrc/kernels/stage1_ring.h
--- a/habdec_amd/csrc/kernels/stage1_ring.h
+++ b/habdec_amd/csrc/kernels/stage1_ring.h
@@ -48,7 +48,7 @@
     uint32_t live;
     uint32_t run_tail;
     uint32_t run_head;
-    uint32_t _pad0;
+    uint32_t gone;
     uint32_t run_q[4];
     uint32_t simd_rank[4];
     uint32_t roles_taken;
@@ -698,9 +698,13 @@
             k[j >> 1].y = (16 * c + j + 1 >= JS && 16 * c + j + 1 < NS) ? taps[16 * c + j + 1] : 0.f;
         }
     };
+    asm volatile("s_waitcnt vmcnt(0)" ::: "memory");
+    asm volatile("" : "+v"(ticket));
+    bool behind_own_store = false;
     for (;;) {
         RSTAMP(2);
-        asm volatile("s_waitcnt vmcnt(0)" ::: "memory");
+        if (behind_own_store && !kWorkerWaitsOwnStore) asm volatile("s_waitcnt vmcnt(1)" ::: "memory");
+        else asm volatile("s_waitcnt vmcnt(0)" ::: "memory");
         asm volatile("" : "+v"(ticket));
         RSTAMP(0);
         r_f32x2 kk[2][2][8];
@@ -788,7 +792,14 @@
         ++n_done;
 #endif
         RSTAMP(1);
-        if (lane >= (uint32_t)HR) a.out[(size_t)cs * a.out_stride + origin + lane - (uint32_t)HR] = make_float2(acc.x, acc.y);
+        {
+            typedef unsigned int w_u32x2 __attribute__((ext_vector_type(2)));
+            const __amdgpu_buffer_rsrc_t out_rs = __builtin_amdgcn_make_buffer_rsrc(const_cast<float2*>(a.out + (size_t)cs * a.out_stride), 0, (int)(rows * 8u), 0x00020000);
+            const uint32_t out_off = lane >= (uint32_t)HR ? (origin + lane - (uint32_t)HR) * 8u : 0x80000000u;
+            const float out_re = acc.x, out_im = acc.y;
+            const w_u32x2 out_v = {__builtin_bit_cast(unsigned int, out_re), __builtin_bit_cast(unsigned int, out_im)};
+            __builtin_amdgcn_raw_buffer_store_b64(out_v, out_rs, (int)out_off, 0, kWtStage1 ? 16 : 0);
+        }
         if (ct + 1 == a.ntiles) {
             const float2* in_s = a.in + (size_t)cs * a.in_stride + (a.n - (uint32_t)(T - 1));
             float2* hout = a.hist_out + (size_t)cs * (T - 1);
@@ -800,6 +811,7 @@
             for (int k = 0; k < NH; ++k) if (lane + 64u * k < (uint32_t)(T - 1)) hout[lane + 64u * k] = h[k];
         }
         if (!more) break;
+        behind_own_store = ct + 1 != a.ntiles;
         cs = ns; ct = nt;
     }
     RSTAMP(2);
diff --git a/habdec_amd/csrc/kernels/tail_body.h b/habdec_amd/csrc/kernels/tail_body.h
--- a/habdec_amd/csrc/kernels/tail_body.h
+++ b/habdec_amd/csrc/kernels/tail_body.h
@@ -454,10 +454,10 @@
                     { float4* c4 = reinterpret_cast<float4*>(cur + fhc + pb + oo); c4[0] = y01; c4[1] = y23; }
                     if (a.fft_in && oo < c.fft_take) {
                         float2* fi = a.fft_in + (size_t)s * kFftBins + c.fft_fill + oo;
-                        if (oo + 3 < c.fft_take && !(c.fft_fill & 1u)) { reinterpret_cast<float4*>(fi)[0] = y01; reinterpret_cast<float4*>(fi)[1] = y23; }
+                        if (oo + 3 < c.fft_take && !(c.fft_fill & 1u)) { store_once<kWtTail>(reinterpret_cast<float4*>(fi), y01); store_once<kWtTail>(reinterpret_cast<float4*>(fi) + 1, y23); }
                         else {
 #pragma unroll
-                            for (int q = 0; q < 4; ++q) if (oo + q < c.fft_take) fi[q] = make_float2(acc[q].x, acc[q].y);
+                            for (int q = 0; q < 4; ++q) if (oo + q < c.fft_take) store_once<kWtTail>(fi + q, make_float2(acc[q].x, acc[q].y));
                         }
                     }
                     done4 = true;
@@ -472,7 +472,7 @@
                         const float2 y = make_float2(acc[q].x, acc[q].y);
                         if (keepF) F[f_old + oo - fbase] = y;
                         cur[fhc + pb + oo] = y;
-                        if (a.fft_in && oo < c.fft_take) a.fft_in[(size_t)s * kFftBins + c.fft_fill + oo] = y;
+                        if (a.fft_in && oo < c.fft_take) store_once<kWtTail>(&a.fft_in[(size_t)s * kFftBins + c.fft_fill + oo], y);
                     }
                 }
             }
@@ -566,10 +566,10 @@
                             float* dm = a.demod + (size_t)s * a.demod_stride + i;
                             const uint32_t pos = end_old + i;
                             const float4 d4 = make_float4(d[0], d[1], d[2], d[3]);
-                            if (nv == 4 && !(i & 3u)) *reinterpret_cast<float4*>(dm) = d4;
+                            if (nv == 4 && !(i & 3u)) store_once<kWtTail>(reinterpret_cast<float4*>(dm), d4);
                             else {
-                                if (nv >= 2) *reinterpret_cast<float2*>(dm) = make_float2(d[0], d[1]); else dm[0] = d[0];
-                                if (nv == 4) *reinterpret_cast<float2*>(dm + 2) = make_float2(d[2], d[3]); else if (nv == 3) dm[2] = d[2];
+                                if (nv >= 2) store_once<kWtTail>(reinterpret_cast<float2*>(dm), make_float2(d[0], d[1])); else store_once<kWtTail>(dm, d[0]);
+                                if (nv == 4) store_once<kWtTail>(reinterpret_cast<float2*>(dm + 2), make_float2(d[2], d[3])); else if (nv == 3) store_once<kWtTail>(dm + 2, d[2]);
                             }
                             if (nv == 4 && !(pos & 3u)) *reinterpret_cast<float4*>(vring + (pos & rmask)) = d4;
                             else {
diff --git a/include/habdec_amd_host.h b/include/habdec_amd_host.h
--- a/include/habdec_amd_host.h
+++ b/include/habdec_amd_host.h
@@ -79,6 +79,8 @@
 void hd_host_tune_tables(float coarse[512], float fine[512]);
 void hd_host_tune_rotate(const float* iq, size_t n, uint32_t phase, uint32_t step, float* out);
 
+double hd_host_step_clock_ms(uint64_t ticks, uint32_t rate_khz);
+
 #ifdef __cplusplus
 }
 #endif
```
